# giesselmann/STRique

Measured on AMD Instinct MI355X. Metric: reads/s for STRique 'count' on 50 kb r9.4 signals, higher is better.
Workload: dtype f32

## Files before the change

strique_amd/csrc/screen_kernels.h:

```cpp
#pragma once
#include <hip/hip_runtime.h>
#include <stdint.h>
#include "align_kernels.h"

#define STRQ_SCREEN_R 14
#define STRQ_SCREEN_S 6
#define STRQ_SCREEN_SEG 4
#define STRQ_SCREEN_CHUNK_COLS 128
#define STRQ_SCREEN_MAX_WINDOWS 4
#define STRQ_SCREEN2_CPL 5
#define STRQ_SCREEN2_LPF 29
#define STRQ_SCREEN2_LANE_B 32

namespace strq {

struct ScreenParams {
    int32_t sc;
    int32_t hh, v;
    int32_t cadd;
    int32_t slack;
    int32_t merge_gap;
    int32_t max_cand;
    int32_t margin;
};

struct ScreenTask {
    const uint8_t* levels;
    const float* table;
    const int32_t* band_lo;
    int32_t* out;
    int32_t tsize;
    int32_t n, m, k, col_off;
    int32_t n_chunks;
    int32_t lane_last;
};

struct Screen2Task {
    const uint8_t* levels;
    const float* table[2];
    const int32_t* band_lo[2];
    int32_t* out[2];
    int32_t tsize[2], k[2];
    int32_t n, col_off, n_chunks;
};

struct ScreenWindows {
    int32_t n_win;
    int32_t lo[STRQ_SCREEN_MAX_WINDOWS], hi[STRQ_SCREEN_MAX_WINDOWS];
    float lower_bound;
    float upper_bound;
    int32_t n_cand;
};

int screen_plan(const AlignParams& p, int samples, int max_n, ScreenParams* sp);
static inline bool screen_flank_ok(int m) { return m >= 2 * STRQ_SCREEN_R && m <= 64 * STRQ_SCREEN_R; }
size_t screen_lds_bytes(int tsize);
int launch_screen(hipStream_t stream, const ScreenTask* tasks, int n_groups, int* queue, const ScreenParams& sp,
                  size_t lds_bytes, int tables_per_cu, int n_cu);
int screen2_plan(const AlignParams& p, int samples, int max_n, int merge, ScreenParams* sp);
static inline bool screen2_flank_ok(int m, int k) { return k >= 1 && k <= STRQ_SCREEN2_LPF * STRQ_SCREEN2_CPL && m == k * STRQ_SCREEN_S; }
size_t screen2_lds_bytes(int tsize_a, int tsize_b);
int launch_screen2(hipStream_t stream, const Screen2Task* tasks, int n_groups, int* queue, const ScreenParams& sp,
                   size_t lds_bytes, int groups_per_cu, int n_cu, int merge);
int launch_screen_windows(hipStream_t stream, const ScreenTask* tasks, int n_groups, const ScreenParams& sp,
                          const int32_t* bound_scaled, ScreenWindows* out, const int32_t* list = nullptr, const int32_t* theta_list = nullptr);

}
```

strique_amd/csrc/screen_kernels.hip:

```cpp
#include "strq_opt.h"
#include <hip/hip_runtime.h>
#include <stdint.h>
#include <stdlib.h>
#include <cmath>
#include "screen_kernels.h"

namespace strq {

namespace {

constexpr int R = STRQ_SCREEN_R, S = STRQ_SCREEN_S, SEG = STRQ_SCREEN_SEG;
constexpr int G = 2, C = 3;
static_assert(R == 14 && S == 6, "class expansion below is written for 14 rows per lane, 6 samples per class");

__device__ __forceinline__ int dpp_shr1(int v, int fill)
{
    return __builtin_amdgcn_update_dpp(fill, v, 0x138, 0xF, 0xF, false);
}
__device__ __forceinline__ int med3i(int a, int lo, int hi)
{
    int r;
    asm("v_med3_i32 %0, %1, %2, %3" : "=v"(r) : "v"(a), "v"(lo), "v"(hi));
    return r;
}
#define STRQ_SCREEN_BIAS 0x00800000
#ifndef STRQ_SCREEN_WPE
#define STRQ_SCREEN_WPE 6
#endif
__device__ __forceinline__ int max3i(int a, int b, int c)
{
    int r;
    asm("v_max3_f32 %0, %1, %2, %3" : "=v"(r) : "v"(a), "v"(b), "v"(c));
    return r;
}
__device__ __forceinline__ int sel_mask(int if0, int if1, uint64_t mask)
{
    int r;
    asm("v_cndmask_b32_e64 %0, %1, %2, %3" : "=v"(r) : "v"(if0), "v"(if1), "s"(mask));
    return r;
}

struct LaneConst { int lo2[C], hi2[C], off[C]; };

struct Screen {
    const char* lds;
    const LaneConst& lc;
    const uint64_t (&pm)[3];
    const int lane, n, hh;
    int T[R], SbotA, upS, potB, cmax;
    int qq;
    int scA[C], scB[C];

    __device__ __forceinline__ void fetch(int q2, int (&sc)[C])
    {
#pragma unroll
        for (int c = 0; c < C; ++c)
            sc[c] = *reinterpret_cast<const uint16_t*>(lds + med3i(q2, lc.lo2[c], lc.hi2[c]) + lc.off[c]);
    }
    __device__ __forceinline__ void advance(int qsrc, int snext, int& qn, int (&nA)[C], int (&nB)[C])
    {
        qn = __builtin_amdgcn_update_dpp(__builtin_amdgcn_readlane(qsrc, snext), qq, 0x138, 0xF, 0xF, false);
        fetch(qn & 0xffff, nA);
        fetch((int)((unsigned)qn >> 16), nB);
    }
    __device__ __forceinline__ void prime(int qcur)
    {
        qq = 0;
        int qn, nA[C], nB[C];
        advance(qcur, 0, qn, nA, nB);
        qq = qn;
#pragma unroll
        for (int c = 0; c < C; ++c) { scA[c] = nA[c]; scB[c] = nB[c]; }
    }
    __device__ __forceinline__ void expand(const int (&sc)[C], int (&rs)[R])
    {
#pragma unroll
        for (int r = 0; r < R; r += G) {
            const int base = r / S, x = (r % S) / G;
            int v;
            if (x == 0 || base + 1 >= C) v = sc[base < C ? base : C - 1];
            else v = sel_mask(sc[base], sc[base + 1], pm[x]);
#pragma unroll
            for (int g = 0; g < G && r + g < R; ++g) rs[r + g] = v;
        }
    }

    template <bool PRED>
    __device__ __forceinline__ void step(int t, int qsrc, int snext)
    {
        const int qn = __builtin_amdgcn_update_dpp(__builtin_amdgcn_readlane(qsrc, snext), qq, 0x138, 0xF, 0xF, false);
        const int potA = potB + hh, potBn = potA + hh;
        const int upA = dpp_shr1(SbotA, potA);
        const int upB = dpp_shr1(T[R - 1], potBn);
        int rsA[R], rsB[R];
        expand(scA, rsA);
        expand(scB, rsB);
        fetch(qn & 0xffff, scA);
        fetch((int)((unsigned)qn >> 16), scB);
        bool act = true, okB = true;
        if constexpr (PRED) { const int jB = 2 * (t - lane), jA = jB - 1; act = (jA >= 1) && (jA <= n); okB = jB <= n; }
        if (act) {
            int ta_prev = upA, ta_prev2 = upS, tb_prev2 = upB;
#pragma unroll
            for (int r = 0; r < R; ++r) {
                const int diagA = r == 0 ? upS : T[r - 1];
                const int ta = max3i(diagA + rsA[r], T[r], ta_prev);
                if (r > 0) {
                    const int tb = max3i(ta_prev2 + rsB[r - 1], ta_prev, tb_prev2);
                    T[r - 1] = tb; tb_prev2 = tb;
                }
                ta_prev2 = ta_prev; ta_prev = ta;
            }
            const int tb = max3i(ta_prev2 + rsB[R - 1], ta_prev, tb_prev2);
            T[R - 1] = tb;
            SbotA = ta_prev;
            upS = upB;
            const int cA = ta_prev - potA + STRQ_SCREEN_BIAS, cB = okB ? tb - potBn + STRQ_SCREEN_BIAS : cA;
            cmax = max3i(cmax, cA, cB);
        }
        potB = potBn;
        qq = qn;
    }
};

__device__ __forceinline__ int load_chunk(const ScreenTask& tk, int chunk, int lane)
{
    const int idx = (chunk * 64 + lane) * 2;
    int a = 0, b = 0;
    if (idx < tk.n) a = tk.levels[idx];
    if (idx + 1 < tk.n) b = tk.levels[idx + 1];
    return (a * 2) | ((b * 2) << 16);
}

}

size_t screen_lds_bytes(int tsize)
{
    return (size_t)((tsize + 1) & ~1) * 2 + 4;
}

__global__ void __attribute__((amdgpu_flat_work_group_size(64 * STRQ_SCREEN_SEG, 64 * STRQ_SCREEN_SEG), amdgpu_waves_per_eu(STRQ_SCREEN_WPE, STRQ_SCREEN_WPE)))
align_screen_kernel(const ScreenTask* __restrict__ tasks, int n_groups, int* __restrict__ queue, ScreenParams sp)
{
    extern __shared__ uint32_t lds_all[];
    __shared__ int next_group;
    const int lane = threadIdx.x & 63, wave = threadIdx.x >> 6;
    const char* ldsb = reinterpret_cast<const char*>(lds_all);
    for (;;) {
        __syncthreads();
        if (threadIdx.x == 0) next_group = atomicAdd(queue, 1);
        __syncthreads();
        const int gi = __builtin_amdgcn_readfirstlane(next_group);
        if (gi >= n_groups) break;
        const ScreenTask& t0 = tasks[(size_t)gi * SEG];
        const int ts = t0.tsize, zero_idx = (ts + 1) & ~1;
        {
            uint16_t* dst = reinterpret_cast<uint16_t*>(lds_all);
            const float scf = (float)sp.sc;
            for (int i = threadIdx.x; i < ts; i += 64 * SEG) dst[i] = (uint16_t)((int)ceilf(t0.table[i] * scf) + sp.cadd);
            if (threadIdx.x == 0) { dst[zero_idx] = 0; dst[zero_idx + 1] = 0; }
        }
        __syncthreads();
        const ScreenTask& tk = tasks[(size_t)gi * SEG + wave];
        if (tk.n <= 0) continue;

        LaneConst lc; uint64_t pm[3];
        {
            const int row0 = lane * R, kbase = row0 / S, phase = row0 % S;
#pragma unroll
            for (int c = 0; c < C; ++c) {
                const int k = kbase + c;
                if (k < tk.k) {
                    const uint32_t d = (uint32_t)tk.band_lo[k];
                    const int lo = (int)(d & 255u), w1 = (int)((d >> 8) & 255u), off = (int)(d >> 16);
                    lc.lo2[c] = lo * 2; lc.hi2[c] = (lo + w1) * 2;
                    lc.off[c] = (off - lo) * 2;
                } else {
                    lc.lo2[c] = 0; lc.hi2[c] = 0; lc.off[c] = zero_idx * 2;
                }
            }
            pm[0] = 0;
#pragma unroll
            for (int x = 1; x < 3; ++x) {
                const uint64_t b = __ballot(phase >= S - x * G);
                const uint32_t lo = __builtin_amdgcn_readfirstlane((int)(uint32_t)b), hi = __builtin_amdgcn_readfirstlane((int)(uint32_t)(b >> 32));
                pm[x] = ((uint64_t)hi << 32) | lo;
            }
        }
        const int lM = (tk.m - 1) / R;
        Screen f{ldsb, lc, pm, lane, tk.n, sp.hh};
        {
#pragma unroll
            for (int r = 0; r < R; ++r) f.T[r] = STRQ_SCREEN_BIAS;
            f.SbotA = STRQ_SCREEN_BIAS; f.upS = STRQ_SCREEN_BIAS;
            f.potB = STRQ_SCREEN_BIAS - 2 * lane * sp.hh;
            f.cmax = STRQ_SCREEN_BIAS;
        }
        const int nsteps = (tk.n + 1) / 2 + 63;
        int qcur = load_chunk(tk, 0, lane);
        f.prime(qcur);
        for (int t0s = 0; t0s < nsteps; t0s += 64) {
            const int qnext = load_chunk(tk, t0s / 64 + 1, lane);
            const bool full = (t0s >= 63) && (2 * (t0s + 64) <= tk.n);
            const int send = nsteps - t0s < 64 ? nsteps - t0s : 64;
            if (full) {
                for (int s = 0; s < 63; ++s) f.template step<false>(t0s + s + 1, qcur, s + 1);
                f.template step<false>(t0s + 64, qnext, 0);
            } else {
                for (int s = 0; s < send; ++s) {
                    const int qsrc = s == 63 ? qnext : qcur, snext = (s + 1) & 63;
                    f.template step<true>(t0s + s + 1, qsrc, snext);
                }
            }
            const int cm = __builtin_amdgcn_readlane(f.cmax, lM) - STRQ_SCREEN_BIAS;
            if (lane == 0) tk.out[t0s / 64] = cm;
            f.cmax = STRQ_SCREEN_BIAS;
            qcur = qnext;
        }
    }
}

namespace {

constexpr int CPL = STRQ_SCREEN2_CPL, LPF = STRQ_SCREEN2_LPF, LB = STRQ_SCREEN2_LANE_B;

struct Lane2Const { int lo2[CPL], hi2[CPL], off[CPL]; };

template <int RPC>
struct Screen2 {
    static constexpr int R2 = RPC * CPL;
    const char* lds;
    const Lane2Const& lc;
    const uint64_t top_mask;
    const int lane, n, hh;
    int T[R2], SbotA, upS, potB, cmax;
    int qq;
    int scA[CPL], scB[CPL];

    __device__ __forceinline__ int score(int q2, int c) const
    {
        return *reinterpret_cast<const uint16_t*>(lds + med3i(q2, lc.lo2[c], lc.hi2[c]) + lc.off[c]);
    }
    __device__ __forceinline__ void prime(int qcur)
    {
        qq = __builtin_amdgcn_update_dpp(__builtin_amdgcn_readlane(qcur, 0), 0, 0x138, 0xF, 0xF, false);
#pragma unroll
        for (int c = 0; c < CPL; ++c) { scA[c] = score(qq & 0xffff, c); scB[c] = score((int)((unsigned)qq >> 16), c); }
    }

    template <bool PRED>
    __device__ __forceinline__ void step(int t, int qsrc, int snext)
    {
        const int qn = __builtin_amdgcn_update_dpp(__builtin_amdgcn_readlane(qsrc, snext), qq, 0x138, 0xF, 0xF, false);
        const int qa = qn & 0xffff, qb = (int)((unsigned)qn >> 16);
        const int potA = potB + hh, potBn = potA + hh;
        const int upA = sel_mask(dpp_shr1(SbotA, potA), potA, top_mask);
        const int upB = sel_mask(dpp_shr1(T[R2 - 1], potBn), potBn, top_mask);
        bool act = true, okB = true;
        if constexpr (PRED) { const int jB = 2 * (t - lane), jA = jB - 1; act = (jA >= 1) && (jA <= n); okB = jB <= n; }
        int ta_prev = upA, ta_prev2 = upS;
        int tb_prev2 = upB;
#pragma unroll
        for (int c = 0; c < CPL; ++c) {
            if (act) {
#pragma unroll
                for (int r = RPC * c; r < RPC * c + RPC; ++r) {
                    const int diagA = r == 0 ? upS : T[r - 1];
                    const int ta = max3i(diagA + scA[c], T[r], ta_prev);
                    if (r > 0) {
                        const int tb = max3i(ta_prev2 + scB[(r - 1) / RPC], ta_prev, tb_prev2);
                        T[r - 1] = tb; tb_prev2 = tb;
                    }
                    ta_prev2 = ta_prev; ta_prev = ta;
                }
                if (c == CPL - 1) {
                    const int tb = max3i(ta_prev2 + scB[c], ta_prev, tb_prev2);
                    T[R2 - 1] = tb;
                    SbotA = ta_prev;
                    upS = upB;
                    const int cA = ta_prev - potA + STRQ_SCREEN_BIAS, cB = okB ? tb - potBn + STRQ_SCREEN_BIAS : cA;
                    cmax = max3i(cmax, cA, cB);
                }
            }
            scA[c] = score(qa, c);
            if (c > 0) scB[c - 1] = score(qb, c - 1);
            if (c == CPL - 1) scB[c] = score(qb, c);
        }
        potB = potBn;
        qq = qn;
    }
};

__device__ __forceinline__ int load_chunk2(const Screen2Task& tk, int chunk, int lane)
{
    const int idx = (chunk * 64 + lane) * 2;
    int a = 0, b = 0;
    if (idx < tk.n) a = tk.levels[idx];
    if (idx + 1 < tk.n) b = tk.levels[idx + 1];
    return (a * 2) | ((b * 2) << 16);
}

template <int RPC>
__device__ __forceinline__ void screen2_body(const Screen2Task* __restrict__ tasks, int n_groups, int* __restrict__ queue, const ScreenParams& sp)
{
    constexpr int R2 = RPC * CPL, MERGE = S / RPC;
    extern __shared__ uint32_t lds_all[];
    __shared__ int next_group;
    const int lane = threadIdx.x & 63, wave = threadIdx.x >> 6;
    const char* ldsb = reinterpret_cast<const char*>(lds_all);
    for (;;) {
        __syncthreads();
        if (threadIdx.x == 0) next_group = atomicAdd(queue, 1);
        __syncthreads();
        const int gi = __builtin_amdgcn_readfirstlane(next_group);
        if (gi >= n_groups) break;
        const Screen2Task& t0 = tasks[(size_t)gi * SEG];
        int base[2], zero_idx[2];
        base[0] = 0; zero_idx[0] = (t0.tsize[0] + 1) & ~1;
        base[1] = zero_idx[0] + 2; zero_idx[1] = base[1] + ((t0.tsize[1] + 1) & ~1);
        {
            uint16_t* dst = reinterpret_cast<uint16_t*>(lds_all);
            const float scf = (float)sp.sc;
#pragma unroll
            for (int f = 0; f < 2; ++f) {
                for (int i = threadIdx.x; i < t0.tsize[f]; i += 64 * SEG) dst[base[f] + i] = (uint16_t)(MERGE * ((int)ceilf(t0.table[f][i] * scf) + sp.cadd));
                if (threadIdx.x == 0) { dst[zero_idx[f]] = 0; dst[zero_idx[f] + 1] = 0; }
            }
        }
        __syncthreads();
        const Screen2Task& tk = tasks[(size_t)gi * SEG + wave];
        if (tk.n <= 0) continue;

        Lane2Const lc;
        const int f = lane >= LB ? 1 : 0, lf = lane - f * LB;
        {
#pragma unroll
            for (int c = 0; c < CPL; ++c) {
                const int k = lf * CPL + c;
                if (lf < LPF && k < tk.k[f]) {
                    const uint32_t d = (uint32_t)tk.band_lo[f][k];
                    const int lo = (int)(d & 255u), w1 = (int)((d >> 8) & 255u), off = (int)(d >> 16);
                    lc.lo2[c] = lo * 2; lc.hi2[c] = (lo + w1) * 2;
                    lc.off[c] = (base[f] + off - lo) * 2;
                } else {
                    lc.lo2[c] = 0; lc.hi2[c] = 0; lc.off[c] = zero_idx[f] * 2;
                }
            }
        }
        const uint64_t top_mask = 1ull | (1ull << LB);
        const int lMa = (tk.k[0] - 1) / CPL, lMb = LB + (tk.k[1] - 1) / CPL;
        Screen2<RPC> s2{ldsb, lc, top_mask, lane, tk.n, sp.hh};
        {
#pragma unroll
            for (int r = 0; r < R2; ++r) s2.T[r] = STRQ_SCREEN_BIAS;
            s2.SbotA = STRQ_SCREEN_BIAS; s2.upS = STRQ_SCREEN_BIAS;
            s2.potB = STRQ_SCREEN_BIAS - 2 * lane * sp.hh;
            s2.cmax = STRQ_SCREEN_BIAS;
        }
        const int nsteps = (tk.n + 1) / 2 + 63;
        int qcur = load_chunk2(tk, 0, lane);
        s2.prime(qcur);
        for (int t0s = 0; t0s < nsteps; t0s += 64) {
            const int qnext = load_chunk2(tk, t0s / 64 + 1, lane);
            const bool full = (t0s >= 63) && (2 * (t0s + 64) <= tk.n);
            const int send = nsteps - t0s < 64 ? nsteps - t0s : 64;
            if (full) {
                for (int s = 0; s < 63; ++s) s2.template step<false>(t0s + s + 1, qcur, s + 1);
                s2.template step<false>(t0s + 64, qnext, 0);
            } else {
                for (int s = 0; s < send; ++s) {
                    const int qsrc = s == 63 ? qnext : qcur, snext = (s + 1) & 63;
                    s2.template step<true>(t0s + s + 1, qsrc, snext);
                }
            }
            const int cma = __builtin_amdgcn_readlane(s2.cmax, lMa) - STRQ_SCREEN_BIAS;
            const int cmb = __builtin_amdgcn_readlane(s2.cmax, lMb) - STRQ_SCREEN_BIAS;
            if (lane == 0) { tk.out[0][t0s / 64] = cma; tk.out[1][t0s / 64] = cmb; }
            s2.cmax = STRQ_SCREEN_BIAS;
            qcur = qnext;
        }
    }
}

}

size_t screen2_lds_bytes(int tsize_a, int tsize_b)
{
    return (size_t)(((tsize_a + 1) & ~1) + 2 + ((tsize_b + 1) & ~1) + 2) * 2;
}

#define STRQ_SCREEN2_ATTR(WPE_) __attribute__((amdgpu_flat_work_group_size(64 * STRQ_SCREEN_SEG, 64 * STRQ_SCREEN_SEG), amdgpu_waves_per_eu(WPE_, WPE_)))
__global__ void STRQ_SCREEN2_ATTR(6) align_screen3_kernel(const Screen2Task* __restrict__ tasks, int n_groups, int* __restrict__ queue, ScreenParams sp) { screen2_body<2>(tasks, n_groups, queue, sp); }
__global__ void STRQ_SCREEN2_ATTR(4) align_screen1_kernel(const Screen2Task* __restrict__ tasks, int n_groups, int* __restrict__ queue, ScreenParams sp) { screen2_body<6>(tasks, n_groups, queue, sp); }

__global__ void __launch_bounds__(256)
screen_windows_kernel(const ScreenTask* __restrict__ tasks, int n_groups, ScreenParams sp,
                      const int32_t* __restrict__ bound_scaled, ScreenWindows* __restrict__ out,
                      const int32_t* __restrict__ list, const int32_t* __restrict__ theta_list)
{
    const int lane = threadIdx.x & 63;
    const int idx = blockIdx.x * (blockDim.x >> 6) + (threadIdx.x >> 6);
    if (idx >= n_groups) return;
    const int g = list ? list[idx] : idx;
    const ScreenTask* tg = tasks + (size_t)g * SEG;
    const int m = tg[0].m, lM = tg[0].lane_last;
    const int shift = -m * sp.v;
    int vmax = 0;
    for (int w = 0; w < SEG; ++w) {
        if (tg[w].n <= 0) continue;
        for (int c = lane; c < tg[w].n_chunks; c += 64) { const int v = tg[w].out[c]; vmax = v > vmax ? v : vmax; }
    }
#pragma unroll
    for (int d = 32; d >= 1; d >>= 1) { const int o = __shfl_xor(vmax, d, 64); vmax = o > vmax ? o : vmax; }
    ScreenWindows r;
    r.n_win = 0; r.n_cand = 0;
    for (int k = 0; k < STRQ_SCREEN_MAX_WINDOWS; ++k) { r.lo[k] = 0; r.hi[k] = 0; }
    const int drop = (sp.margin > 0 ? sp.margin : m) + 2 * sp.slack;
    int theta = theta_list ? theta_list[idx] : vmax - drop;
    if (!theta_list && sp.max_cand > 0) {
        auto count_at = [&](int t) {
            int n = 0;
            for (int w = 0; w < SEG; ++w) {
                if (tg[w].n <= 0) continue;
                for (int c = lane; c < tg[w].n_chunks; c += 64) n += tg[w].out[c] >= t;
            }
#pragma unroll
            for (int d = 32; d >= 1; d >>= 1) n += __shfl_xor(n, d, 64);
            return n;
        };
        if (count_at(theta) > sp.max_cand) {
            int lo = theta, hi = vmax;
            while (hi - lo > 1) {
                const int mid = lo + (hi - lo) / 2;
                if (count_at(mid) > sp.max_cand) lo = mid; else hi = mid;
            }
            theta = hi;
        }
    }
    r.upper_bound = (float)(vmax + shift + sp.slack) / (float)sp.sc;
    auto scan = [&](int th, bool store) -> int {
        int nw = 0, last_hi = -(1 << 30), ncand = 0;
        for (int w = 0; w < SEG; ++w) {
            if (tg[w].n <= 0) continue;
            for (int c0 = 0; c0 < tg[w].n_chunks; c0 += 64) {
                const int c1 = c0 + lane;
                const bool cand = c1 < tg[w].n_chunks && tg[w].out[c1] >= th;
                uint64_t mask = __ballot(cand);
                while (mask) {
                    const int bit = __builtin_ctzll(mask); mask &= mask - 1;
                    const int c = c0 + bit;
                    ++ncand;
                    int lo = 128 * c - 2 * lM + 1, hi = 128 * c - 2 * lM + 128;
                    if (lo < 1) lo = 1;
                    if (hi > tg[w].n) hi = tg[w].n;
                    if (hi < lo) continue;
                    lo += tg[w].col_off; hi += tg[w].col_off;
                    if (nw > 0 && lo <= last_hi + sp.merge_gap) {
                        if (hi > last_hi) last_hi = hi;
                        if (store) {
                            const int k = nw <= STRQ_SCREEN_MAX_WINDOWS ? nw - 1 : STRQ_SCREEN_MAX_WINDOWS - 1;
                            if (hi > r.hi[k]) r.hi[k] = hi;
                            if (lo < r.lo[k]) r.lo[k] = lo;
                        }
                    } else {
                        ++nw; last_hi = hi;
                        if (store) {
                            if (nw <= STRQ_SCREEN_MAX_WINDOWS) { r.lo[nw - 1] = lo; r.hi[nw - 1] = hi; }
                            else if (hi > r.hi[STRQ_SCREEN_MAX_WINDOWS - 1]) r.hi[STRQ_SCREEN_MAX_WINDOWS - 1] = hi;
                        }
                    }
                }
            }
        }
        if (store) r.n_cand = ncand;
        return nw;
    };
    if (!theta_list && sp.max_cand > 0 && scan(theta, false) > STRQ_SCREEN_MAX_WINDOWS) {
        int lo = theta, hi = vmax;
        while (hi - lo > 1) {
            const int mid = lo + (hi - lo) / 2;
            if (scan(mid, false) > STRQ_SCREEN_MAX_WINDOWS) lo = mid; else hi = mid;
        }
        theta = hi;
    }
    {
        const double lb = (double)(theta + shift + sp.slack) / (double)sp.sc;
        float lbf = (float)lb;
        if ((double)lbf < lb) {
            int32_t bits = __float_as_int(lbf);
            bits = lbf > 0.0f ? bits + 1 : (lbf < 0.0f ? bits - 1 : 1);
            lbf = __int_as_float(bits);
        }
        r.lower_bound = lbf;
    }
    const bool ok = theta + shift > 0 && theta + shift > bound_scaled[g];
    if (ok) {
        int nw = scan(theta, true);
        if (nw > STRQ_SCREEN_MAX_WINDOWS) nw = STRQ_SCREEN_MAX_WINDOWS;
        for (int a = 1; a < nw; ++a)
            for (int b = a; b > 0 && r.lo[b] < r.lo[b - 1]; --b) {
                const int tl = r.lo[b], th = r.hi[b]; r.lo[b] = r.lo[b - 1]; r.hi[b] = r.hi[b - 1]; r.lo[b - 1] = tl; r.hi[b - 1] = th;
            }
        int kept = nw > 0 ? 1 : 0;
        for (int a = 1; a < nw; ++a) {
            if (r.lo[a] <= r.hi[kept - 1] + 1) { if (r.hi[a] > r.hi[kept - 1]) r.hi[kept - 1] = r.hi[a]; }
            else { r.lo[kept] = r.lo[a]; r.hi[kept] = r.hi[a]; ++kept; }
        }
        for (int a = kept; a < STRQ_SCREEN_MAX_WINDOWS; ++a) { r.lo[a] = 0; r.hi[a] = 0; }
        r.n_win = kept;
    }
    if (lane == 0) out[idx] = r;
}

int screen_plan(const AlignParams& p, int samples, int max_n, ScreenParams* sp)
{
    if (strq::opt("STRQ_NO_SCREEN")) return 0;
    if (samples != S) return 0;
    if (!(p.open_h == p.ext_h && p.open_v == p.ext_v)) return 0;
    if (!(p.dist_min >= 0.0f) || !(p.ext_h < 0.0f) || !(p.ext_v < 0.0f) || !(p.dist_offset > 0.0f) || !(p.dist_min <= p.dist_offset)) return 0;
    for (int sc = 1024; sc >= 16; sc >>= 1) {
        const double hh = -(double)p.ext_h * sc, v = -(double)p.ext_v * sc, smax = std::ceil((double)p.dist_offset * sc);
        if (hh != (double)(long)hh || v != (double)(long)v) continue;
        if (hh < 1 || smax + v + hh > 65000.0) continue;
        const double top = 64.0 * R * (smax + v) + ((double)max_n + 256.0) * hh + smax + v + hh + (double)STRQ_SCREEN_BIAS;
        if (top > 2.0e9) continue;
        sp->sc = sc; sp->hh = (int)hh; sp->v = (int)v; sp->cadd = (int)(hh + v);
        {
            const double rows = 64.0 * R, maxval = rows * (double)p.dist_offset;
            double p2 = 1.0; while (p2 < maxval) p2 *= 2.0;
            const double adds = rows * (1.0 + (double)p.dist_offset / -(double)p.ext_h);
            const double e = adds * p2 / 16777216.0;
            if (!(e < 1.0e4)) continue;
            sp->slack = ((int)std::ceil(e) + 1) * sc;
        }
        sp->merge_gap = 3072; sp->margin = 0; sp->max_cand = 0;
        return 1;
    }
    return 0;
}

int screen2_plan(const AlignParams& p, int samples, int max_n, int merge, ScreenParams* sp)
{
    if (merge != 1 && merge != 3) return 0;
    if (!screen_plan(p, samples, max_n, sp)) return 0;
    while (sp->sc >= 16) {
        const double smax = std::ceil((double)p.dist_offset * sp->sc);
        if ((double)merge * (smax + sp->cadd) <= 65000.0) return 1;
        if ((sp->hh & 1) || (sp->v & 1)) return 0;
        sp->slack = (sp->slack / sp->sc) * (sp->sc / 2);
        sp->sc /= 2; sp->hh /= 2; sp->v /= 2; sp->cadd = sp->hh + sp->v;
    }
    return 0;
}

int launch_screen2(hipStream_t stream, const Screen2Task* tasks, int n_groups, int* queue, const ScreenParams& sp,
                   size_t lds_bytes, int groups_per_cu, int n_cu, int merge)
{
    if (n_groups <= 0) return 0;
    if (merge != 3 && merge != 1) return 2;
    auto kern = merge == 3 ? align_screen3_kernel : align_screen1_kernel;
    if (merge == 1 && groups_per_cu > 4) groups_per_cu = 4;
    if (groups_per_cu > 6) groups_per_cu = 6;
    (void)hipFuncSetAttribute((const void*)kern, hipFuncAttributeMaxDynamicSharedMemorySize, (int)lds_bytes);
    hipLaunchKernelGGL(kern, dim3(groups_per_cu * n_cu), dim3(64 * SEG), lds_bytes, stream, tasks, n_groups, queue, sp);
    return hipGetLastError() == hipSuccess ? 0 : 1;
}

int launch_screen(hipStream_t stream, const ScreenTask* tasks, int n_groups, int* queue, const ScreenParams& sp,
                  size_t lds_bytes, int tables_per_cu, int n_cu)
{
    if (n_groups <= 0) return 0;
    (void)hipFuncSetAttribute((const void*)align_screen_kernel, hipFuncAttributeMaxDynamicSharedMemorySize, (int)lds_bytes);
    hipLaunchKernelGGL(align_screen_kernel, dim3(tables_per_cu * n_cu), dim3(64 * SEG), lds_bytes, stream, tasks, n_groups, queue, sp);
    return hipGetLastError() == hipSuccess ? 0 : 1;
}

int launch_screen_windows(hipStream_t stream, const ScreenTask* tasks, int n_groups, const ScreenParams& sp,
                          const int32_t* bound_scaled, ScreenWindows* out, const int32_t* list, const int32_t* theta_list)
{
    if (n_groups <= 0) return 0;
    hipLaunchKernelGGL(screen_windows_kernel, dim3((n_groups + 3) / 4), dim3(256), 0, stream, tasks, n_groups, sp, bound_scaled, out, list, theta_list);
    return hipGetLastError() == hipSuccess ? 0 : 1;
}

}
```

strique_amd/csrc/strq_align_api.hip:

```cpp
#include <hip/hip_runtime.h>
#include <algorithm>
#include <cmath>
#include <climits>
#include <cstring>
#include <cstdlib>
#include <time.h>
#include <unistd.h>
#include <map>
#include <mutex>
#include <string>
#include <tuple>
#include <numeric>
#include <vector>
#include "../../include/strique_hip.h"
#include "strq_ctx.h"
#include "align_kernels.h"
#include "lut_kernels.h"
#include "align_generic.h"

using namespace strq;

#define STRQ_DBG(...) do { if (strq::opt("STRQ_DEBUG")) { fprintf(stderr, "[strq] " __VA_ARGS__); fprintf(stderr, "\n"); fflush(stderr); } } while (0)

namespace strq {

static thread_local const strq_ctx* t_cur_ctx = nullptr;
static std::mutex g_opt_mu;
static std::map<std::string, std::string> g_opts;
CtxScope::CtxScope(const strq_ctx* c) : prev(t_cur_ctx) { t_cur_ctx = c; }
CtxScope::~CtxScope() { t_cur_ctx = prev; }
const char* opt(const char* key)
{
    static thread_local std::string ring[8];
    static thread_local unsigned ring_pos = 0;
    auto keep = [&](const std::string& v) -> const char* {
        if (v.empty()) return nullptr;
        std::string& slot = ring[ring_pos++ & 7u];
        slot = v;
        return slot.c_str();
    };
    if (t_cur_ctx) {
        std::lock_guard<std::mutex> lk(t_cur_ctx->options_mu);
        auto it = t_cur_ctx->options.find(key);
        if (it != t_cur_ctx->options.end()) return keep(it->second);
    }
    {
        std::lock_guard<std::mutex> lk(g_opt_mu);
        auto it = g_opts.find(key);
        if (it != g_opts.end()) return keep(it->second);
    }
    return getenv(key);
}

float host_cell_score(const AlignParams& p, float h, float v)
{
    const float d = h > v ? h - v : v - h;
    const float s = p.dist_offset - (float)std::pow((double)d, 1.2);
    return s > p.dist_min ? s : p.dist_min;
}

void host_col0(const AlignParams& p, int m, float* out)
{
    const float NINF = -3.4028234663852886e38f / 2;
    out[0] = 0.0f;
    float vprev = NINF, sprev = 0.0f;
    for (int i = 1; i <= m; ++i) {
        const float ext = vprev + p.ext_v, opn = sprev + p.open_v;
        const float v = ext >= opn ? ext : opn;
        out[i] = v; vprev = v; sprev = v;
    }
}

struct BatchIn {
    int64_t n_align, n_reads;
    const uint8_t* levels; const int64_t* read_off; const float* level_val;
    const int32_t* align_read; const float* flank; const int64_t* flank_off; int32_t samples;
};
struct BatchOut { float* score; int64_t* j_end; int64_t* j0; int32_t* rec; };


static const int hard_cap = 1 << 16;
static const int trace_wpb = 8;

struct Piece { int col_off, n; size_t ck; };

static int cut(int n, int segs, int ov, Piece* out)
{
    int use = segs;
    while (use > 1 && (ov <= 0 || (long)n < (long)(use + 1) * ov)) --use;
    const long len = use > 1 ? ((long)n + (long)(use - 1) * ov + use - 1) / use : n;
    long o = 0;
    for (int k = 0; k < segs; ++k) {
        if (k >= use) { out[k].col_off = 0; out[k].n = 0; continue; }
        const long start = k == 0 ? 0 : o - ov;
        long end = k == use - 1 ? n : start + len; if (end > n) end = n;
        out[k].col_off = (int)start; out[k].n = (int)(end - start);
        o = end;
    }
    return use;
}

static int packed_dwords(int entries) { return (((2 * entries + 3) & ~3) + entries + 3) / 4; }

struct Launch { int R, NS, tables, first, count, first_task, first_up, lds_floats, packed, segs; bool known_last_row; };

struct CorePlan {
    CorePlan(strq_ctx* c_, const AlignCoreIn& in_, AlignCoreOut& out_) : c(c_), in(in_), out(out_), nb(in_.nb), S(in_.samples), st(c_->stream) {}
    strq_ctx* c;
    const AlignCoreIn& in;
    AlignCoreOut& out;
    const int nb, S;
    const hipStream_t st;

    bool collapsed = false, allow_pack = false, ov_fixed = false, scr_forced = false, mode_fine = false, mode_coarse = false;
    int seg_want = 0, max_tables = 8, max_waves = 16, ov_cap = 8192;
    std::map<std::pair<int, int>, int> ov_of_m;

    std::vector<size_t> cls_off, col0_off, bnd_off;
    std::vector<int> J0, NJ;
    std::vector<int> job_align, job_k0, job_k;
    std::vector<size_t> tab_off, desc_off;
    int nj = 0, max_k = 0;
    std::vector<float> h_cls;
    std::vector<LutJob> jobs;
    std::vector<LutInfo> info;
    std::vector<int> tab_total;

    std::vector<ScreenWindows> wins;
    bool screen2_ran = false;
    std::vector<int> g2_of;
    ScreenTask* d_st2 = nullptr;
    int32_t* d_bound2 = nullptr;
    ScreenParams sp2{};
    double coarse_cols = 0, coarse_all = 0;

    std::vector<char> packed;
    std::vector<int> overlap, segs_of;
    std::vector<Launch> launches;
    int n_up = 0, max_ns = 1, r2_cap = 0, qi = STRQ_QUEUE_FIRST;
    size_t n_tasks = 0, safe0 = 0, r2_0 = 0;
    std::vector<Piece> pieces, safe;
    std::vector<float> min_score;
    std::vector<char> two_round;
    bool any_two_round = false;
    std::vector<size_t> ck_up;
    std::vector<AlignTask> tasks;
    AlignTask *d_tasks = nullptr, *d_heads = nullptr;
    AlignResult *d_seg = nullptr, *d_res = nullptr, *d_seg_safe = nullptr;
    int32_t* d_pick = nullptr;
    float* d_min_score = nullptr;
    int *d_redo = nullptr, *d_redo_count = nullptr;
};

static int overlap_for(CorePlan& p, int m, int ov_worst, int redo_weight = 1)
{
    strq_ctx* c = p.c;
    if (p.ov_fixed || c->score_fracs.size() < 64 || c->mean_n <= 0) return std::min(ov_worst, p.ov_cap);
    auto it = p.ov_of_m.find(std::make_pair(m, redo_weight));
    if (it != p.ov_of_m.end()) return it->second;
    const std::vector<float>& f = c->score_fracs;
    double best_cost = 0; int best_ov = std::min(ov_worst, p.ov_cap);
    for (int ov = 1024; ; ov += 512) {
        if (ov > ov_worst) ov = ov_worst;
        const float need = align_segment_min_score(c->ap, m, ov) / ((float)m * c->ap.dist_offset) + 0.01f;
        const double redo = (double)(std::lower_bound(f.begin(), f.end(), need) - f.begin()) / (double)f.size();
        const double cost = 3.0 * ov / c->mean_n + redo_weight * redo * (1.0 + 3.0 * ov_worst / c->mean_n);
        if (best_cost == 0 || cost < best_cost) { best_cost = cost; best_ov = ov; }
        if (ov >= ov_worst) break;
    }
    p.ov_of_m[std::make_pair(m, redo_weight)] = best_ov;
    STRQ_DBG("overlap for %d-row flanks: %d columns (worst case %d; previous sub-batch: median score fraction %.3f, mean read %.0f samples)", m, best_ov, ov_worst, f[f.size() / 2], c->mean_n);
    return best_ov;
}

static int tables_for(const CorePlan& p, int dwords, int segs)
{
    int t = std::min(p.max_tables, (160 * 1024 - 64) / (std::max(dwords, 1) * 4));
    if (segs > 1) t = std::min(t, p.max_waves / segs);
    return t;
}

static void pause_after_fail(int& pause, int& fail)
{
    pause = std::min(256, 8 << std::min(fail, 5));
    ++fail;
}

static int upload_inputs(CorePlan& p)
{
    strq_ctx* c = p.c; const AlignCoreIn& in = p.in; AlignCoreOut& out = p.out;
    const int nb = p.nb, S = p.S;
    hipStream_t st = p.st;
    size_t cls_tot = 0, col0_tot = 0, rec_tot = 0, tab_tot = 0, bnd_floats = 0, desc_tot = 0;
    p.cls_off.assign(nb, 0); p.col0_off.assign(nb, 0); p.bnd_off.assign(nb, 0);
    std::map<const float*, size_t> cls_of_flank; std::map<int, size_t> col0_of_m;
    std::vector<int> cls_first, col0_first;
    out.rec_off.assign(nb, 0);
    p.J0.assign(nb, 0); p.NJ.assign(nb, 0);
    for (int i = 0; i < nb; ++i) {
        auto fc = cls_of_flank.find(in.flank[i]);
        if (fc == cls_of_flank.end()) { fc = cls_of_flank.emplace(in.flank[i], cls_tot).first; cls_tot += in.k[i]; cls_first.push_back(i); }
        p.cls_off[i] = fc->second;
        auto f0 = col0_of_m.find(in.m[i]);
        if (f0 == col0_of_m.end()) { f0 = col0_of_m.emplace(in.m[i], col0_tot).first; col0_tot += in.m[i] + 1; col0_first.push_back(i); }
        p.col0_off[i] = f0->second;
        p.J0[i] = (int)p.job_align.size();
        p.NJ[i] = in.k[i] > STRQ_LUT_MAX_K ? in.NS[i] : 1;
        for (int sidx = 0; sidx < p.NJ[i]; ++sidx) {
            int k0 = 0, kn = in.k[i];
            if (p.NJ[i] > 1) {
                const int row0 = sidx * 64 * in.R[i], rows = std::min(64 * in.R[i], in.m[i] - row0);
                k0 = row0 / S; kn = (row0 + rows - 1) / S - k0 + 1;
            }
            p.job_align.push_back(i); p.job_k0.push_back(k0); p.job_k.push_back(kn);
            p.desc_off.push_back(desc_tot); desc_tot += kn;
            p.tab_off.push_back(tab_tot); tab_tot += STRQ_TABLE_SLOT_FLOATS(kn);
            p.max_k = std::max(p.max_k, kn);
        }
        out.rec_off[i] = rec_tot; rec_tot += in.m[i];
        p.bnd_off[i] = bnd_floats; if (in.NS[i] > 1) bnd_floats += (size_t)(in.NS[i] - 1) * 2 * ((size_t)in.n[i] + 2);
    }
    const int nj = p.nj = (int)p.job_align.size();
    out.rec_total = rec_tot;
    p.h_cls.assign(cls_tot, 0.0f);
    std::vector<float> h_col0(col0_tot);
    for (int i : cls_first) {
        const float* f = in.flank[i];
        for (int kk = 0; kk < in.k[i]; ++kk) p.h_cls[p.cls_off[i] + kk] = f[(size_t)kk * S];
    }
    for (int i : col0_first) host_col0(c->ap, in.m[i], &h_col0[p.col0_off[i]]);
    STRQ_HIP(c, c->flank_cls.reserve(cls_tot * 4));
    STRQ_HIP(c, c->col0.reserve(col0_tot * 4));
    STRQ_HIP(c, c->band_lo.reserve(desc_tot * 4));
    STRQ_HIP(c, c->tables.reserve(tab_tot * 4));
    STRQ_HIP(c, c->tables3.reserve(tab_tot * 3 + (size_t)nj * 8 + 64));
    STRQ_HIP(c, c->bnd.reserve(bnd_floats * 4 + 256));
    STRQ_HIP(c, c->rec.reserve(rec_tot * 4 + 256));
    STRQ_HIP(c, c->lutinfo.reserve((size_t)nj * (sizeof(LutJob) + sizeof(LutInfo))));
    STRQ_HIP(c, c->hard.reserve((size_t)hard_cap * (sizeof(HardEntry) + 4) + 64));
    STRQ_HIP(c, c->queue.reserve(STRQ_QUEUE_BYTES));
    STRQ_HIP(c, hipMemcpyAsync(c->flank_cls.p, p.h_cls.data(), cls_tot * 4, hipMemcpyHostToDevice, st));
    STRQ_HIP(c, hipMemcpyAsync(c->col0.p, h_col0.data(), col0_tot * 4, hipMemcpyHostToDevice, st));
    STRQ_HIP(c, hipMemsetAsync(c->queue.p, 0, STRQ_QUEUE_BYTES, st));
    return STRQ_OK;
}

static int build_tables(CorePlan& p)
{
    strq_ctx* c = p.c; const AlignCoreIn& in = p.in;
    const int nb = p.nb, nj = p.nj;
    hipStream_t st = p.st;
    std::vector<LutJob>& jobs = p.jobs;
    std::vector<LutInfo>& info = p.info;
    jobs.resize(nj);
    LutJob* d_jobs = c->lutinfo.as<LutJob>();
    LutInfo* d_info = reinterpret_cast<LutInfo*>(d_jobs + nj);
    for (int j = 0; j < nj; ++j) {
        const int i = p.job_align[j];
        jobs[j].level_val = in.d_level_val + (size_t)in.read[i] * 256;
        jobs[j].cls_val = c->flank_cls.as<float>() + p.cls_off[i] + p.job_k0[j];
        jobs[j].table = c->tables.as<float>() + p.tab_off[j];
        jobs[j].table3 = c->tables3.as<uint8_t>() + p.tab_off[j] * 3 + (size_t)j * 8 - (p.tab_off[j] * 3 + (size_t)j * 8) % 4;
        jobs[j].band_lo = c->band_lo.as<int32_t>() + p.desc_off[j];
        jobs[j].k = p.job_k[j]; jobs[j].pad_ = 0;
    }
    STRQ_HIP(c, hipMemcpyAsync(d_jobs, jobs.data(), (size_t)nj * sizeof(LutJob), hipMemcpyHostToDevice, st));
    HardEntry* d_hard = c->hard.as<HardEntry>();
    float* d_hard_vals = reinterpret_cast<float*>(d_hard + hard_cap);
    int* d_hard_count = c->queue.as<int>();
    STRQ_HIP(c, hipEventRecord(c->ev[0], st));
    if (launch_lut_build(st, d_jobs, d_info, nj, p.max_k, d_hard, d_hard_count, hard_cap, c->ap)) { c->err = "lut launch failed"; return STRQ_ERR_DEVICE; }
    STRQ_HIP(c, hipEventRecord(c->ev[1], st));
    if (in.after_tables) { const int arc = in.after_tables(); if (arc) return arc; }
    info.resize(nj);
    int hard_count = 0;
    STRQ_HIP(c, hipMemcpyAsync(info.data(), d_info, (size_t)nj * sizeof(LutInfo), hipMemcpyDeviceToHost, st));
    STRQ_HIP(c, hipMemcpyAsync(&hard_count, d_hard_count, 4, hipMemcpyDeviceToHost, st));
    STRQ_HIP(c, hipStreamSynchronize(st));
    STRQ_DBG("lut done nb=%d hard=%d floats0=%d", nb, hard_count, info[0].total);
    if (strq::opt("STRQ_DEBUG")) { int hist[9] = {0}; for (int i = 0; i < nj; ++i) hist[std::min(8, info[i].need / 8)]++; STRQ_DBG("band need histogram (x8 levels): %d %d %d %d %d %d %d %d %d", hist[0], hist[1], hist[2], hist[3], hist[4], hist[5], hist[6], hist[7], hist[8]); }
    if (strq::opt("STRQ_DEBUG")) { long tot = 0; int mx = 0; for (int i = 0; i < nj; ++i) { tot += info[i].total; mx = std::max(mx, info[i].total); } STRQ_DBG("table floats: mean %.0f max %d (k=%d)", (double)tot / nj, mx, in.k[0]); }
    if (hard_count > hard_cap) { c->err = "too many borderline table entries"; return STRQ_ERR_DEVICE; }
    bool any_rebuild = false;
    for (int j = 0; j < nj; ++j) any_rebuild |= info[j].n_hard < 0;
    auto level_vals_of = [&](int read, float* dst) -> int {
        STRQ_HIP(c, hipMemcpy(dst, in.d_level_val + (size_t)read * 256, 256 * 4, hipMemcpyDeviceToHost));
        return STRQ_OK;
    };
    if (hard_count > 0) {
        std::vector<HardEntry> he(hard_count); std::vector<float> hv(hard_count);
        STRQ_HIP(c, hipMemcpy(he.data(), d_hard, (size_t)hard_count * sizeof(HardEntry), hipMemcpyDeviceToHost));
        float lv[256]; int last_read = -1;
        for (int i = 0; i < hard_count; ++i) {
            const int rd = in.read[p.job_align[he[i].job]];
            if (rd != last_read) { const int rc = level_vals_of(rd, lv); if (rc) return rc; last_read = rd; }
            hv[i] = host_cell_score(c->ap, lv[he[i].level], p.h_cls[p.cls_off[p.job_align[he[i].job]] + p.job_k0[he[i].job] + he[i].k]);
        }
        STRQ_HIP(c, hipMemcpyAsync(d_hard_vals, hv.data(), (size_t)hard_count * 4, hipMemcpyHostToDevice, st));
        if (launch_lut_patch(st, d_jobs, d_hard, d_hard_vals, hard_count)) { c->err = "patch launch failed"; return STRQ_ERR_DEVICE; }
        STRQ_HIP(c, hipStreamSynchronize(st));
    }
    if (any_rebuild) for (int j = 0; j < nj; ++j) if (info[j].n_hard < 0) {
        const int kk = p.job_k[j], i = p.job_align[j];
        std::vector<float> tab((size_t)kk * 256); std::vector<int32_t> blo(kk);
        float lv[256];
        { const int rc = level_vals_of(in.read[i], lv); if (rc) return rc; }
        for (int x = 0; x < kk; ++x) {
            float* row = &tab[(size_t)x * 256];
            for (int q = 0; q < 256; ++q) row[q] = host_cell_score(c->ap, lv[q], p.h_cls[p.cls_off[i] + p.job_k0[j] + x]);
            blo[x] = (int32_t)((255u << 8) | ((uint32_t)(x * 256) << 16));
        }
        STRQ_HIP(c, hipMemcpy(jobs[j].table, tab.data(), tab.size() * 4, hipMemcpyHostToDevice));
        STRQ_HIP(c, hipMemcpy(jobs[j].band_lo, blo.data(), (size_t)kk * 4, hipMemcpyHostToDevice));
        info[j].total = kk * 256;
    }
    p.tab_total.assign(nb, 0);
    for (int j = 0; j < nj; ++j) p.tab_total[p.job_align[j]] = std::max(p.tab_total[p.job_align[j]], info[j].total);
    p.out.n_hard = hard_count;
    return STRQ_OK;
}

static void read_switches(CorePlan& p)
{
    const strq_ctx* c = p.c;
    p.collapsed = p.S == 6 && c->ap.open_h == c->ap.ext_h && c->ap.open_v == c->ap.ext_v;
    if (const char* e = strq::opt("STRQ_SEG")) { const int v = atoi(e); if (v >= 1 && v <= 4) p.seg_want = v; }
    if (const char* e = strq::opt("STRQ_TABLES")) { const int v = atoi(e); if (v >= 1 && v <= 8) p.max_tables = v; }
    if (const char* e = strq::opt("STRQ_MAX_WAVES")) { const int v = atoi(e); if (v >= 4 && v <= 16) p.max_waves = v; }
    p.allow_pack = p.collapsed && !strq::opt("STRQ_NO_PACK");
    if (const char* e = strq::opt("STRQ_OVERLAP")) { const int v = atoi(e); p.ov_cap = v > 0 ? v : (1 << 30); p.ov_fixed = true; }
    p.scr_forced = strq::opt("STRQ_SCREEN_ALWAYS") != nullptr;
    const char* mode_opt = strq::opt("STRQ_SCREEN_MODE");
    p.mode_fine = mode_opt && std::strcmp(mode_opt, "fine") == 0;
    p.mode_coarse = mode_opt && std::strcmp(mode_opt, "coarse") == 0;
}


struct ScreenJob {
    int flanks = 1;
    std::vector<int> al;
    std::vector<ScreenTask> views;
    std::vector<Screen2Task> t2;
    std::vector<int32_t> bound;
    std::vector<size_t> out_off;
    size_t out_words = 0, lds_bytes = 0;
    double steps = 0;
};

struct ScreenRules {
    int merge;
    int groups_per_cu;
    const char* lds_err;
    bool below_bound_free;
    bool count_untaken;
    bool judge;
    double max_cols;
    int* pause; int* fail;
};

static void screen_tasks(CorePlan& p, const ScreenParams& sp, ScreenJob& j)
{
    constexpr int SSEG = STRQ_SCREEN_SEG;
    const AlignCoreIn& in = p.in;
    const int F = j.flanks, ng = (int)j.al.size() / F;
    if (F == 2) j.t2.resize((size_t)ng * SSEG);
    j.views.resize(j.al.size() * SSEG);
    j.bound.resize(j.al.size());
    j.out_off.assign(j.al.size() * SSEG, 0);
    for (int g = 0; g < ng; ++g) {
        const int* a = &j.al[(size_t)g * F];
        const int n = in.n[a[0]];
        const int m_big = F == 2 ? std::max(in.m[a[0]], in.m[a[1]]) : in.m[a[0]];
        const int ov_worst = align_segment_overlap(p.c->ap, m_big), ov_s = overlap_for(p, m_big, ov_worst, 16);
        Piece pc[SSEG];
        const int used = cut(n, SSEG, ov_s, pc);
        j.lds_bytes = std::max(j.lds_bytes, F == 2 ? screen2_lds_bytes(p.info[p.J0[a[0]]].total, p.info[p.J0[a[1]]].total) : screen_lds_bytes(p.info[p.J0[a[0]]].total));
        for (int f = 0; f < F; ++f)
            j.bound[(size_t)g * F + f] = used <= 1 ? INT32_MIN / 2 : (ov_s >= ov_worst ? 0 : (int32_t)std::ceil((double)align_segment_min_score(p.c->ap, in.m[a[f]], ov_s) * sp.sc));
        for (int w = 0; w < SSEG; ++w) {
            Screen2Task t; std::memset(&t, 0, sizeof(t));
            t.levels = in.d_levels + in.read_off[in.read[a[0]]] + pc[w].col_off;
            t.n = pc[w].n; t.col_off = pc[w].col_off;
            t.n_chunks = pc[w].n > 0 ? (align_num_steps(pc[w].n) + 63) / 64 : 0;
            for (int f = 0; f < F; ++f) {
                const LutJob& job = p.jobs[p.J0[a[f]]];
                t.table[f] = job.table; t.band_lo[f] = job.band_lo; t.tsize[f] = p.info[p.J0[a[f]]].total; t.k[f] = in.k[a[f]];
                ScreenTask v; std::memset(&v, 0, sizeof(v));
                v.n = pc[w].n; v.m = in.m[a[f]]; v.k = in.k[a[f]]; v.col_off = pc[w].col_off; v.n_chunks = t.n_chunks;
                if (F == 2) v.lane_last = f * STRQ_SCREEN2_LANE_B + (in.k[a[f]] - 1) / STRQ_SCREEN2_CPL;
                else { v.levels = t.levels; v.table = t.table[0]; v.band_lo = t.band_lo[0]; v.tsize = t.tsize[0]; v.lane_last = (v.m - 1) / STRQ_SCREEN_R; }
                j.out_off[((size_t)g * F + f) * SSEG + w] = j.out_words; j.out_words += (size_t)t.n_chunks;
                j.views[((size_t)g * F + f) * SSEG + w] = v;
            }
            if (pc[w].n > 0) j.steps += align_num_steps(pc[w].n);
            if (F == 2) j.t2[(size_t)g * SSEG + w] = t;
        }
    }
}

static int run_screen(CorePlan& p, ScreenJob& j, const ScreenParams& sp, const ScreenRules& r)
{
    constexpr int SSEG = STRQ_SCREEN_SEG;
    strq_ctx* c = p.c; const AlignCoreIn& in = p.in;
    hipStream_t st = p.st;
    const int nv = (int)j.al.size();
    if (j.lds_bytes > 160 * 1024 - 64) { c->err = r.lds_err; return STRQ_ERR_UNSUPPORTED; }
    const int groups = std::max(1, std::min(r.groups_per_cu, (int)((160 * 1024 - 64) / j.lds_bytes)));
    auto aligned = [](size_t bytes) { return (bytes + 255) & ~(size_t)255; };
    const size_t t2_bytes = aligned(j.t2.size() * sizeof(Screen2Task)), task_bytes = aligned(j.views.size() * sizeof(ScreenTask));
    const size_t bound_bytes = aligned((size_t)nv * 4), win_bytes = aligned((size_t)nv * sizeof(ScreenWindows));
    STRQ_HIP(c, c->screen.reserve(t2_bytes + task_bytes + bound_bytes + win_bytes + j.out_words * 4 + 256));
    char* base = c->screen.as<char>();
    Screen2Task* d_t2 = reinterpret_cast<Screen2Task*>(base);
    ScreenTask* d_st = reinterpret_cast<ScreenTask*>(base + t2_bytes);
    int32_t* d_bound = reinterpret_cast<int32_t*>(base + t2_bytes + task_bytes);
    ScreenWindows* d_win = reinterpret_cast<ScreenWindows*>(base + t2_bytes + task_bytes + bound_bytes);
    int32_t* d_out = reinterpret_cast<int32_t*>(base + t2_bytes + task_bytes + bound_bytes + win_bytes);
    for (size_t x = 0; x < j.views.size(); ++x) j.views[x].out = d_out + j.out_off[x];
    if (j.flanks == 2)
        for (int v = 0; v < nv; ++v) for (int w = 0; w < SSEG; ++w) j.t2[(size_t)(v / 2) * SSEG + w].out[v % 2] = j.views[(size_t)v * SSEG + w].out;
    if (j.flanks == 2) STRQ_HIP(c, hipMemcpyAsync(d_t2, j.t2.data(), j.t2.size() * sizeof(Screen2Task), hipMemcpyHostToDevice, st));
    STRQ_HIP(c, hipMemcpyAsync(d_st, j.views.data(), j.views.size() * sizeof(ScreenTask), hipMemcpyHostToDevice, st));
    STRQ_HIP(c, hipMemcpyAsync(d_bound, j.bound.data(), (size_t)nv * 4, hipMemcpyHostToDevice, st));
    STRQ_HIP(c, hipEventRecord(c->ev[5], st));
    int* queue = c->queue.as<int>() + STRQ_QUEUE_FIRST - 1;
    if (j.flanks == 2) {
        if (launch_screen2(st, d_t2, nv / 2, queue, sp, j.lds_bytes, groups, c->n_cu, r.merge)) { c->err = "coarse screen launch failed"; return STRQ_ERR_DEVICE; }
    } else {
        if (launch_screen(st, d_st, nv, queue, sp, j.lds_bytes, groups, c->n_cu)) { c->err = "screen launch failed"; return STRQ_ERR_DEVICE; }
    }
    STRQ_HIP(c, hipEventRecord(c->ev[6], st));
    if (launch_screen_windows(st, d_st, nv, sp, d_bound, d_win)) { c->err = "screen windows launch failed"; return STRQ_ERR_DEVICE; }
    std::vector<ScreenWindows> hw((size_t)nv);
    STRQ_HIP(c, hipMemcpyAsync(hw.data(), d_win, hw.size() * sizeof(ScreenWindows), hipMemcpyDeviceToHost, st));
    STRQ_HIP(c, hipStreamSynchronize(st));
    c->screen_ran = true; c->screen_mode_last = r.merge > 1 ? 2 : 1; c->coarse_merge_last = r.merge;
    if (const char* path = strq::opt("STRQ_SCREEN_DUMP")) {
        std::vector<int32_t> ho(j.out_words);
        STRQ_HIP(c, hipMemcpy(ho.data(), d_out, j.out_words * 4, hipMemcpyDeviceToHost));
        if (FILE* fp = fopen(path, "wb")) {
            const int32_t hdr[8] = {nv, sp.sc, sp.hh, sp.v, j.flanks, SSEG, sp.slack, r.merge};
            fwrite(hdr, 4, 8, fp);
            for (int v = 0; v < nv; ++v) {
                const int32_t gh[4] = {j.al[v], j.al[v], j.bound[v], j.views[(size_t)v * SSEG].lane_last};
                fwrite(gh, 4, 4, fp);
                for (int w = 0; w < SSEG; ++w) {
                    const ScreenTask& t = j.views[(size_t)v * SSEG + w];
                    const int32_t th[4] = {t.col_off, t.n, t.m, t.n_chunks};
                    fwrite(th, 4, 4, fp);
                    fwrite(ho.data() + (t.out - d_out), 4, (size_t)t.n_chunks, fp);
                }
                fwrite(&hw[(size_t)v], sizeof(ScreenWindows), 1, fp);
            }
            fclose(fp);
        }
    }
    if (const char* e = strq::opt("STRQ_SCREEN_TEST_RAISE")) {
        const float up = (float)atof(e);
        for (auto& w : hw) w.lower_bound += up;
    }
    int windowed = 0, heavy = 0, below_bound = 0; double cols = 0, all = 0;
    for (int v = 0; v < nv; ++v) {
        const int al = j.al[v];
        const ScreenWindows& w = hw[(size_t)v];
        c->screen_stats[1] += 1; c->screen_stats[7] += w.n_cand;
        double mine = in.n[al];
        if (w.n_win > 0) {
            p.wins[al] = w; c->screen_stats[2] += 1; ++windowed; mine = 0;
            for (int k = 0; k < w.n_win; ++k) { c->screen_stats[4] += w.hi[k] - w.lo[k] + 1; mine += w.hi[k] - w.lo[k] + 1 + 4096; }
        } else {
            c->screen_stats[3] += 1;
            if (w.n_cand == 0) { ++below_bound; if (r.below_bound_free) mine = 0; }
        }
        all += in.n[al]; cols += mine; heavy += mine > 4 * 32768.0;
    }
    if (r.count_untaken) c->screen_stats[3] += p.nb - nv;
    c->screen_stats[5] += j.steps; c->screen_stats[6] = sp.sc;
    if (j.flanks == 2) {
        p.screen2_ran = true;
        p.d_st2 = d_st; p.d_bound2 = d_bound; p.sp2 = sp;
        for (int v = 0; v < nv; ++v) p.g2_of[j.al[v]] = v;
        p.coarse_cols = cols; p.coarse_all = all;
    }
    if (r.judge && nv >= 64) {
        if (below_bound * 10 > nv && !p.ov_fixed) c->score_fracs.clear();
        else if (windowed < 0.9 * (nv - (p.ov_fixed ? 0 : below_bound)) || cols > r.max_cols * all || (long)heavy * 100 > 2L * nv) pause_after_fail(*r.pause, *r.fail);
        else *r.fail = 0;
    }
    STRQ_DBG("screen (%d flanks per wave, merge %d): %d alignments, scale %d, margin %.0f, %d groups per CU, LDS %zu bytes: %d with windows (%d below the cold-start bound), %.2f %% of the columns, %d heavy -> pause %d",
             j.flanks, r.merge, nv, sp.sc, (double)sp.margin / sp.sc, groups, j.lds_bytes, windowed, below_bound, 100.0 * cols / std::max(1.0, all), heavy, *r.pause);
    return STRQ_OK;
}

static int screen_two_flank(CorePlan& p, int merge, int max_n)
{
    strq_ctx* c = p.c; const AlignCoreIn& in = p.in;
    const int nb = p.nb;
    ScreenParams sp;
    if (!screen2_plan(c->ap, p.S, max_n, merge, &sp)) return STRQ_OK;
    const bool fine_rules = merge == 1;
    int min_n = fine_rules ? 65536 : 28672, groups = 6;
    if (const char* e = strq::opt("STRQ_SCREEN_MIN_N")) min_n = atoi(e);
    if (const char* e = strq::opt("STRQ_SCREEN2_GROUPS")) { const int v = atoi(e); if (v >= 1 && v <= 8) groups = v; }
    std::map<int, std::vector<int>> by_read;
    for (int i = 0; i < nb; ++i)
        if (in.NS[i] == 1 && p.NJ[i] == 1 && in.n[i] >= min_n && screen2_flank_ok(in.m[i], in.k[i])) by_read[in.read[i]].push_back(i);
    std::vector<std::pair<int, int>> pairs;
    for (auto& kv : by_read) {
        const std::vector<int>& v = kv.second;
        if (v.size() == 2) { pairs.emplace_back(v[0], v[1]); continue; }
        for (size_t x = 0; x + 1 < v.size(); ++x)
            if (!(v[x] & 1) && v[x + 1] == v[x] + 1) { pairs.emplace_back(v[x], v[x + 1]); ++x; }
    }
    std::stable_sort(pairs.begin(), pairs.end(), [&](const std::pair<int, int>& x, const std::pair<int, int>& y) { return in.n[x.first] > in.n[y.first]; });
    const int ngr = (int)pairs.size();
    if (ngr == 0 || 2 * ngr < (nb * 9) / 10) return STRQ_OK;
    sp.margin = (int32_t)std::lround((double)c->coarse_margin * (merge == 3 ? 1.3 : 1.0) * sp.sc);
    if (const char* e = strq::opt("STRQ_SCREEN2_MARGIN")) sp.margin = (int32_t)std::lround(atof(e) * sp.sc);
    sp.max_cand = 8;
    if (const char* e = strq::opt("STRQ_SCREEN2_MAX_CAND")) sp.max_cand = atoi(e);
    if (fine_rules) { sp.margin = 0; sp.max_cand = 0; }
    ScreenJob j;
    j.flanks = 2;
    for (const auto& pr : pairs) { j.al.push_back(pr.first); j.al.push_back(pr.second); }
    screen_tasks(p, sp, j);
    ScreenRules r;
    r.merge = merge; r.groups_per_cu = groups;
    r.lds_err = "score tables do not fit LDS (coarse screen)";
    r.below_bound_free = !p.ov_fixed; r.count_untaken = true;
    if (fine_rules) { r.judge = !p.scr_forced; r.max_cols = 0.15; r.pause = &c->screen_pause; r.fail = &c->screen_fail; }
    else { r.judge = !p.mode_coarse && !p.scr_forced; r.max_cols = 0.30; r.pause = &c->coarse_pause; r.fail = &c->coarse_fail; }
    return run_screen(p, j, sp, r);
}

static int screen_one_flank(CorePlan& p, const ScreenParams& sp)
{
    strq_ctx* c = p.c; const AlignCoreIn& in = p.in;
    int min_n = 65536;
    if (const char* e = strq::opt("STRQ_SCREEN_MIN_N")) min_n = atoi(e);
    std::vector<int> sel;
    for (int i = 0; i < p.nb; ++i)
        if (in.NS[i] == 1 && p.NJ[i] == 1 && in.n[i] >= min_n && screen_flank_ok(in.m[i]) && in.k[i] * p.S == in.m[i]) sel.push_back(i);
    std::stable_sort(sel.begin(), sel.end(), [&](int x, int y) { return in.n[x] > in.n[y]; });
    if (sel.empty()) return STRQ_OK;
    ScreenJob j;
    j.al = sel;
    screen_tasks(p, sp, j);
    ScreenRules r;
    r.merge = 0; r.groups_per_cu = 6;
    r.lds_err = "score table does not fit LDS (screen)";
    r.below_bound_free = false; r.count_untaken = false;
    r.judge = true; r.max_cols = 0.10; r.pause = &c->screen_pause; r.fail = &c->screen_fail;
    return run_screen(p, j, sp, r);
}

static int run_screens(CorePlan& p)
{
    strq_ctx* c = p.c; const AlignCoreIn& in = p.in;
    const int nb = p.nb;
    p.wins.resize(nb);
    c->screen_ran = false;
    STRQ_HIP(c, hipEventRecord(c->ev[2], p.st));
    int max_n = 0;
    for (int i = 0; i < nb; ++i) max_n = std::max(max_n, in.n[i]);
    c->screen_mode_last = 0;
    const int coarse_merge = 3;
    p.g2_of.assign(nb, -1);
    for (int attempt = 0; attempt < 2 && !p.screen2_ran; ++attempt) {
        int merge = coarse_merge;
        if (attempt == 0) {
            if (!p.collapsed || p.mode_fine || strq::opt("STRQ_NO_SCREEN")) continue;
            if (c->coarse_pause > 0 && !p.mode_coarse && !p.scr_forced) { --c->coarse_pause; continue; }
        } else {
            if (!p.collapsed || strq::opt("STRQ_NO_SCREEN") || (c->screen_pause > 0 && !p.scr_forced)) continue;
            merge = 1;
        }
        const int rc = screen_two_flank(p, merge, max_n);
        if (rc) return rc;
    }
    if (p.screen2_ran) return STRQ_OK;
    if (p.collapsed && c->screen_pause > 0 && !p.scr_forced) {
        --c->screen_pause; c->screen_stats[3] += nb;
        return STRQ_OK;
    }
    ScreenParams sp;
    if (p.collapsed && screen_plan(c->ap, p.S, max_n, &sp)) return screen_one_flank(p, sp);
    return STRQ_OK;
}

static int plan_launches(CorePlan& p)
{
    strq_ctx* c = p.c; const AlignCoreIn& in = p.in; AlignCoreOut& out = p.out;
    const int nb = p.nb;
    std::vector<ScreenWindows>& wins = p.wins;
    static const double rate[5][2] = {{0, 0}, {1.017, 0.941}, {0.79, 0.862}, {0.85, 0.85}, {0.69, 0.80}};
    p.packed.assign(nb, 0); p.overlap.assign(nb, 0); p.segs_of.assign(nb, 1);
    std::vector<char> segmentable(nb, 0);
    const bool force_pack = strq::opt("STRQ_PACK") != nullptr;
    int class_count[5] = {0, 0, 0, 0, 0};
    for (int i = 0; i < nb; ++i) {
        segmentable[i] = p.collapsed && in.NS[i] == 1;
        p.overlap[i] = segmentable[i] ? align_segment_overlap(c->ap, in.m[i]) : 0;
        const bool can_pack = p.allow_pack && in.NS[i] == 1 && p.info[p.J0[i]].packed && p.info[p.J0[i]].n_hard == 0;
        int best_s = 1, best_p = can_pack ? 1 : 0;
        if (segmentable[i]) {
            const double l = overlap_for(p, in.m[i], p.overlap[i]);
            double best_cost = 0;
            for (int sgs : {1, 2, 3, 4}) {
                if (p.seg_want ? sgs != p.seg_want : sgs == 3) continue;
                if (sgs > 1 && !p.seg_want && (l <= 0 || in.n[i] < (sgs + 1) * l)) continue;
                for (int pk = 0; pk < 2; ++pk) {
                    if ((pk && !can_pack) || (force_pack && can_pack && !pk)) continue;
                    const double cost = (in.n[i] + (sgs - 1) * l) * rate[sgs][pk];
                    if (best_cost == 0 || cost < best_cost) { best_cost = cost; best_s = sgs; best_p = pk; }
                }
            }
        }
        if (wins[i].n_win > 0) {
            ScreenWindows& w = wins[i];
            while (w.n_win < STRQ_SCREEN_MAX_WINDOWS) {
                int widest = 0;
                for (int k2 = 1; k2 < w.n_win; ++k2) if (w.hi[k2] - w.lo[k2] > w.hi[widest] - w.lo[widest]) widest = k2;
                if (w.hi[widest] - w.lo[widest] < 16384) break;
                const int mid = w.lo[widest] + (w.hi[widest] - w.lo[widest]) / 2;
                for (int k2 = w.n_win; k2 > widest + 1; --k2) { w.lo[k2] = w.lo[k2 - 1]; w.hi[k2] = w.hi[k2 - 1]; }
                w.lo[widest + 1] = mid + 1; w.hi[widest + 1] = w.hi[widest]; w.hi[widest] = mid;
                ++w.n_win;
            }
            const int nw = w.n_win;
            best_s = p.seg_want >= nw ? p.seg_want : (nw <= 2 ? nw : 4); best_p = 0;
        }
        p.segs_of[i] = best_s; p.packed[i] = (char)best_p;
        ++class_count[best_s];
    }
    std::vector<int>& segs_of = p.segs_of;
    if (!p.seg_want && !c->screen_ran) {
        int few = 2 * c->n_cu;
        if (const char* e = strq::opt("STRQ_CLASS_MIN")) few = atoi(e);
        if (class_count[4] && class_count[4] < few) { for (int i = 0; i < nb; ++i) if (segs_of[i] == 4) { segs_of[i] = 2; if (wins[i].n_win > 2) wins[i].n_win = 0; } class_count[2] += class_count[4]; class_count[4] = 0; }
        if (class_count[2] && class_count[2] < few && class_count[1]) { for (int i = 0; i < nb; ++i) if (segs_of[i] == 2) { segs_of[i] = 1; if (wins[i].n_win > 1) wins[i].n_win = 0; } class_count[1] += class_count[2]; class_count[2] = 0; }
    }
    std::map<std::tuple<int, int, int, int, int>, std::vector<int>> groups;
    for (int i = 0; i < nb; ++i) {
        const int w = tables_for(p, p.packed[i] ? packed_dwords(p.tab_total[i]) : p.tab_total[i], segs_of[i]);
        if (w < 1) { c->err = "score table does not fit LDS"; return STRQ_ERR_UNSUPPORTED; }
        groups[std::make_tuple(in.R[i], in.NS[i], -segs_of[i], -w, p.packed[i] ? 0 : 1)].push_back(i);
    }
    const int min_rounds = 4;
    for (auto it = groups.begin(); it != groups.end();) {
        auto nx = std::next(it);
        const int w = -std::get<3>(it->first);
        const bool same_kind = nx != groups.end() && std::get<0>(nx->first) == std::get<0>(it->first) && std::get<1>(nx->first) == std::get<1>(it->first)
                               && std::get<2>(nx->first) == std::get<2>(it->first)
                               && !(std::get<4>(it->first) == 1 && std::get<4>(nx->first) == 0);
        if (same_kind && (long)it->second.size() < (long)min_rounds * w * c->n_cu) {
            nx->second.insert(nx->second.end(), it->second.begin(), it->second.end());
            it = groups.erase(it);
        } else ++it;
    }
    out.order.clear(); out.order.reserve(nb);
    for (auto& g : groups) {
        auto& v = g.second;
        auto work = [&](int x) {
            if (wins[x].n_win <= 0) return (long)in.n[x];
            long w = 0;
            for (int k = 0; k < wins[x].n_win; ++k) w += wins[x].hi[k] - wins[x].lo[k] + 1 + 4096;
            return w;
        };
        std::stable_sort(v.begin(), v.end(), [&](int x, int y) { return work(x) > work(y); });
        const int NS = std::get<1>(g.first);
        const int pk = std::get<4>(g.first) == 0;
        int lds_floats = 0;
        for (int i : v) lds_floats = std::max(lds_floats, pk ? packed_dwords(p.tab_total[i]) : p.tab_total[i]);
        const int segs = -std::get<2>(g.first);
        const int tables = std::min(-std::get<3>(g.first), tables_for(p, lds_floats, segs));
        if (tables < 1) { c->err = "score table does not fit LDS"; return STRQ_ERR_UNSUPPORTED; }
        bool known = std::get<0>(g.first) == 14;
        for (int i : v) known = known && in.m[i] == 870;
        p.launches.push_back({std::get<0>(g.first), NS, tables, (int)out.order.size(), (int)v.size(), (int)p.n_tasks, 0, lds_floats, pk, segs, known});
        out.order.insert(out.order.end(), v.begin(), v.end());
        p.n_tasks += (size_t)v.size() * segs;
        if (NS > 1) p.n_up += (int)v.size() * (NS - 1);
    }
    { size_t up = p.n_tasks; for (auto& L : p.launches) if (L.NS > 1) { L.first_up = (int)up; up += (size_t)L.count * (L.NS - 1); } }
    return STRQ_OK;
}

static int cut_pieces(CorePlan& p)
{
    strq_ctx* c = p.c; const AlignCoreIn& in = p.in; const AlignCoreOut& out = p.out;
    const int nb = p.nb;
    const size_t n_tasks = p.n_tasks;
    p.safe0 = n_tasks + p.n_up + (size_t)nb;
    p.pieces.resize(n_tasks); p.safe.resize(n_tasks);
    p.min_score.assign(nb, -INFINITY);
    p.two_round.assign(p.launches.size(), 0);
    p.ck_up.assign(nb, 0);
    size_t ck_floats = 0;
    for (size_t li = 0; li < p.launches.size(); ++li) {
        auto& L = p.launches[li];
        for (int x = 0; x < L.count; ++x) {
            const int pos = L.first + x, i = out.order[pos];
            const int n = in.n[i], R = in.R[i], ov = p.overlap[i];
            const size_t per_ckpt = (size_t)STRQ_CKPT_FIELDS(R) * 64;
            Piece* pf = &p.pieces[(size_t)L.first_task + (size_t)x * L.segs];
            Piece* ps = &p.safe[(size_t)L.first_task + (size_t)x * L.segs];
            cut(n, L.segs, ov, ps);
            const int ov_fast = overlap_for(p, in.m[i], ov);
            if (p.wins[i].n_win > 0) {
                const ScreenWindows& w = p.wins[i];
                const int ov_w = std::min(ov > 0 ? ov : (1 << 30), align_overlap_for_score(c->ap, in.m[i], w.lower_bound));
                for (int k = 0; k < L.segs; ++k) {
                    if (k < w.n_win) { const int start = std::max(0, w.lo[k] - 1 - ov_w); pf[k].col_off = start; pf[k].n = w.hi[k] - start; }
                    else { pf[k].col_off = 0; pf[k].n = 0; }
                }
                p.min_score[pos] = std::max(w.lower_bound, align_segment_min_score(c->ap, in.m[i], ov_w));
                p.two_round[li] = 1;
            } else if (L.segs > 1 && ov_fast < ov && cut(n, L.segs, ov_fast, pf) > 1) {
                p.min_score[pos] = align_segment_min_score(c->ap, in.m[i], ov_fast);
                p.two_round[li] = 1;
            } else {
                for (int k = 0; k < L.segs; ++k) pf[k] = ps[k];
            }
            for (int k = 0; k < L.segs; ++k) {
                pf[k].ck = ps[k].ck = ck_floats;
                ck_floats += (size_t)align_num_ckpts(std::max(pf[k].n, ps[k].n)) * per_ckpt;
            }
            if (L.NS > 1) { p.ck_up[i] = ck_floats; ck_floats += (size_t)(L.NS - 1) * align_num_ckpts(n) * per_ckpt; }
        }
    }
    for (char t : p.two_round) p.any_two_round |= t != 0;
    const size_t n_all_tasks = p.safe0 + (p.any_two_round ? n_tasks : 0);
    STRQ_HIP(c, c->ckpt.reserve(ck_floats * 4 + 256));
    p.r2_cap = p.screen2_ran ? std::max(1024, std::min(nb, 8192)) : 0;
    p.r2_0 = n_all_tasks;
    STRQ_HIP(c, c->tasks.reserve((n_all_tasks + (size_t)p.r2_cap * 4) * sizeof(AlignTask)));
    STRQ_HIP(c, c->results.reserve((2 * n_tasks + nb) * sizeof(AlignResult) + (size_t)nb * 12 + p.launches.size() * 4 + 256));
    p.tasks.resize(n_all_tasks);
    p.d_tasks = c->tasks.as<AlignTask>();
    p.d_heads = p.d_tasks + n_tasks + p.n_up;
    p.d_seg = c->results.as<AlignResult>();
    p.d_res = p.d_seg + n_tasks;
    p.d_seg_safe = p.d_res + nb;
    p.d_pick = reinterpret_cast<int32_t*>(p.d_seg_safe + n_tasks);
    p.d_min_score = reinterpret_cast<float*>(p.d_pick + nb);
    p.d_redo = reinterpret_cast<int*>(p.d_min_score + nb);
    p.d_redo_count = p.d_redo + nb;
    return STRQ_OK;
}

static int write_tasks(CorePlan& p)
{
    strq_ctx* c = p.c; const AlignCoreIn& in = p.in; AlignCoreOut& out = p.out;
    const int nb = p.nb, S = p.S;
    hipStream_t st = p.st;
    const size_t n_tasks = p.n_tasks, n_up = p.n_up, safe0 = p.safe0;
    std::vector<AlignTask>& tasks = p.tasks;
    for (auto& L : p.launches) {
        for (int x = 0; x < L.count; ++x) {
            const int pos = L.first + x, i = out.order[pos];
            const int R = in.R[i], M = in.m[i];
            AlignTask base; std::memset(&base, 0, sizeof(base));
            base.levels = in.d_levels + in.read_off[in.read[i]];
            base.rec = c->rec.as<int32_t>() + out.rec_off[i];
            base.n = in.n[i]; base.n_full = in.n[i]; base.m_total = M;
            auto strip = [&](int row0, int rows, size_t ck, int sidx) {
                AlignTask t = base;
                const int j = p.NJ[i] > 1 ? p.J0[i] + sidx : p.J0[i];
                const int k0 = row0 / S, k1 = (row0 + rows - 1) / S;
                t.row0 = row0; t.m = rows; t.k = k1 - k0 + 1; t.tsize = p.info[j].total;
                t.table = p.jobs[j].table; t.table3 = p.jobs[j].table3; t.band_lo = p.jobs[j].band_lo + (k0 - p.job_k0[j]);
                t.col0 = c->col0.as<float>() + p.col0_off[i] + row0;
                t.ckpt = c->ckpt.as<float>() + ck;
                return t;
            };
            tasks[n_tasks + n_up + pos] = strip(0, M, 0, 0);
            if (L.NS == 1) {
                for (int k = 0; k < L.segs; ++k) {
                    const size_t ti = (size_t)L.first_task + (size_t)x * L.segs + k;
                    AlignTask t = strip(0, M, p.pieces[ti].ck, 0);
                    t.levels += p.pieces[ti].col_off; t.n = p.pieces[ti].n; t.col_off = p.pieces[ti].col_off;
                    tasks[ti] = t;
                    if (p.any_two_round) {
                        AlignTask u = strip(0, M, p.safe[ti].ck, 0);
                        u.levels += p.safe[ti].col_off; u.n = p.safe[ti].n; u.col_off = p.safe[ti].col_off;
                        tasks[safe0 + ti] = u;
                    }
                }
            } else {
                const int rows_s = 64 * R;
                const size_t ck_strip = (size_t)align_num_ckpts(in.n[i]) * STRQ_CKPT_FIELDS(R) * 64;
                float* bnd = c->bnd.as<float>() + p.bnd_off[i];
                const size_t bnd_stride = 2 * ((size_t)in.n[i] + 2);
                for (int sidx = 0; sidx < L.NS; ++sidx) {
                    const bool last = sidx == L.NS - 1;
                    const int row0 = sidx * rows_s, rows = last ? M - row0 : rows_s;
                    const size_t slot = last ? (size_t)L.first_task + x : (size_t)L.first_up + (size_t)sidx * L.count + x;
                    AlignTask t = strip(row0, rows, last ? p.pieces[(size_t)L.first_task + x].ck : p.ck_up[i] + (size_t)sidx * ck_strip, sidx);
                    if (sidx > 0) { t.bnd_in = bnd + (size_t)(sidx - 1) * bnd_stride; t.up = p.d_tasks + L.first_up + (size_t)(sidx - 1) * L.count + x; }
                    if (!last) t.bnd_out = bnd + (size_t)sidx * bnd_stride;
                    tasks[slot] = t;
                    if (last && p.any_two_round) tasks[safe0 + slot] = t;
                }
            }
        }
    }
    STRQ_HIP(c, hipMemcpyAsync(p.d_tasks, tasks.data(), tasks.size() * sizeof(AlignTask), hipMemcpyHostToDevice, st));
    STRQ_HIP(c, hipMemsetAsync(p.d_seg, 0, (2 * n_tasks + nb) * sizeof(AlignResult), st));
    if (p.any_two_round) {
        STRQ_HIP(c, hipMemcpyAsync(p.d_min_score, p.min_score.data(), (size_t)nb * 4, hipMemcpyHostToDevice, st));
        STRQ_HIP(c, hipMemsetAsync(p.d_redo_count, 0, p.launches.size() * 4, st));
    }
    size_t scratch_words = 0;
    for (auto& L : p.launches) scratch_words = std::max(scratch_words, align_trace_scratch_words_per_wave(L.R));
    STRQ_HIP(c, c->scratch.reserve(scratch_words * 8 * (size_t)c->n_cu * trace_wpb));
    out.n_launches = 0; out.wave_steps = 0; out.columns = 0;
    for (size_t t = 0; t < n_tasks + n_up; ++t) if (tasks[t].n > 0) { out.wave_steps += align_num_steps(tasks[t].n); out.columns += tasks[t].n; }
    if (!p.launches.empty()) {
        const Launch& L = p.launches.back(); out.segs = L.segs; out.tables = L.tables; out.packed = L.packed; out.rows_per_lane = L.R;
        const int i = out.order[L.first];
        out.overlap_worst = p.overlap[i]; out.overlap_first = L.segs > 1 ? overlap_for(p, in.m[i], p.overlap[i]) : 0;
        const bool seg_kernel = L.NS == 1 && p.collapsed;
        const int32_t g[8] = {L.segs, L.tables, seg_kernel ? align_segments_wpe(L.segs, L.tables) : 0, L.R, L.packed, out.overlap_first, out.overlap_worst, (int32_t)p.launches.size()};
        std::memcpy(c->geometry, g, sizeof(g));
    }
    return STRQ_OK;
}

static int run_forward(CorePlan& p)
{
    strq_ctx* c = p.c; AlignCoreOut& out = p.out;
    const int S = p.S;
    hipStream_t st = p.st;
    const std::vector<Launch>& launches = p.launches;
    for (auto& L : launches) p.max_ns = std::max(p.max_ns, L.NS);
    if ((size_t)STRQ_QUEUE_FIRST + launches.size() * ((size_t)p.max_ns + 2) + 16 > (size_t)STRQ_QUEUE_SLOTS) {
        c->err = "too many distinct (flank shape, table size) groups in one batch"; return STRQ_ERR_UNSUPPORTED;
    }
    bool side = false;
    std::vector<hipStream_t> lstream(launches.size(), st);
    if (c->screen_ran && launches.size() > 1 && p.max_ns == 1 && p.collapsed) {
        side = true;
        if (!c->ev_fork) STRQ_HIP(c, hipEventCreateWithFlags(&c->ev_fork, hipEventDisableTiming));
        STRQ_HIP(c, hipEventRecord(c->ev_fork, st));
        size_t biggest = 0;
        for (size_t li = 1; li < launches.size(); ++li) if (launches[li].count > launches[biggest].count) biggest = li;
        if (!c->side_stream) { STRQ_HIP(c, hipStreamCreateWithFlags(&c->side_stream, hipStreamNonBlocking)); STRQ_HIP(c, hipEventCreateWithFlags(&c->side_join, hipEventDisableTiming)); }
        STRQ_HIP(c, hipStreamWaitEvent(c->side_stream, c->ev_fork, 0));
        lstream[biggest] = c->side_stream;
    }
    for (int level = 0; level < p.max_ns; ++level) {
        for (size_t lidx = 0; lidx < launches.size(); ++lidx) {
            const Launch& L = launches[lidx];
            hipStream_t lst = lstream[lidx];
            if (level >= L.NS) continue;
            STRQ_DBG("forward launch R=%d strips=%d slice dwords=%d packed=%d level=%d count=%d tables/CU=%d segments=%d", L.R, L.NS, L.lds_floats, L.packed, level, L.count, L.tables, L.segs);
            int rc;
            if (L.NS == 1 && p.collapsed) {
                rc = launch_align_segments(lst, L.R, S, p.d_tasks + L.first_task, p.d_seg + L.first_task, L.count, L.segs, c->queue.as<int>() + p.qi,
                                           c->ap, L.lds_floats, L.tables, c->n_cu, L.packed, nullptr, nullptr, L.known_last_row);
            } else {
                const bool last = level == L.NS - 1;
                const AlignTask* dt = last ? p.d_tasks + L.first_task : p.d_tasks + L.first_up + (size_t)level * L.count;
                const int mode = (level > 0 ? 1 : 0) | (last ? 0 : 2);
                rc = launch_align(st, L.R, S, dt, p.d_seg + L.first_task, L.count, c->queue.as<int>() + p.qi, c->ap, L.lds_floats, L.tables, c->n_cu,
                                  c->scratch.as<uint64_t>(), 0, mode, L.packed);
            }
            if (rc) { c->err = "align launch failed"; return STRQ_ERR_DEVICE; }
            ++p.qi; ++out.n_launches;
        }
    }
    if (side) {
        STRQ_HIP(c, hipEventRecord(c->side_join, c->side_stream));
        STRQ_HIP(c, hipStreamWaitEvent(st, c->side_join, 0));
    }
    for (size_t li = 0; li < launches.size(); ++li) {
        const Launch& L = launches[li];
        int* redo = p.d_redo + L.first; int* cnt = p.d_redo_count + li;
        if (launch_align_combine(st, p.d_tasks + L.first_task, p.d_seg + L.first_task, L.count, L.segs, p.d_res + L.first, p.d_pick + L.first, L.first_task,
                                 nullptr, nullptr, p.two_round[li] ? p.d_min_score + L.first : nullptr, redo, cnt,
                                 c->redo_total.p ? c->redo_total.as<unsigned int>() : nullptr)) { c->err = "combine launch failed"; return STRQ_ERR_DEVICE; }
    }
    return STRQ_OK;
}

struct Look2 { int pos, i, g2; float b1; };

static void keep_whole_read(const CorePlan& p, std::vector<std::vector<int>>& redo_keep, int pos)
{
    for (size_t li = 0; li < p.launches.size(); ++li) {
        const Launch& L = p.launches[li];
        if (pos >= L.first && pos < L.first + L.count) redo_keep[li].push_back(pos - L.first);
    }
}

static int look2_run(CorePlan& p, const std::vector<Look2>& l2, std::vector<std::vector<int>>& redo_keep)
{
    strq_ctx* c = p.c; const AlignCoreIn& in = p.in; AlignCoreOut& out = p.out;
    const int nb = p.nb, S = p.S;
    hipStream_t st = p.st;
    const ScreenParams& sp2 = p.sp2;
    const int n2 = (int)l2.size();
    const size_t o_list = 0, o_theta = o_list + (size_t)n2 * 4, o_win = (o_theta + (size_t)n2 * 4 + 15) & ~(size_t)15,
                 o_pos = o_win + (size_t)n2 * sizeof(ScreenWindows), o_seg = (o_pos + (size_t)n2 * 4 + 15) & ~(size_t)15,
                 o_res = o_seg + (size_t)n2 * 4 * sizeof(AlignResult), o_pick = o_res + (size_t)n2 * sizeof(AlignResult), o_end = o_pick + (size_t)n2 * 4;
    STRQ_HIP(c, c->misc.reserve(o_end + 256));
    char* mb = c->misc.as<char>();
    std::vector<int32_t> h_list((size_t)n2), h_theta((size_t)n2), h_pos((size_t)n2);
    for (int k2 = 0; k2 < n2; ++k2) {
        const Look2& e = l2[(size_t)k2];
        h_list[(size_t)k2] = e.g2; h_pos[(size_t)k2] = e.pos;
        const double b1s = std::floor((double)e.b1 * sp2.sc);
        h_theta[(size_t)k2] = (int32_t)std::max(-2.0e9, std::min(2.0e9, b1s + (double)in.m[e.i] * sp2.v - (double)sp2.slack));
    }
    STRQ_HIP(c, hipMemcpyAsync(mb + o_list, h_list.data(), (size_t)n2 * 4, hipMemcpyHostToDevice, st));
    STRQ_HIP(c, hipMemcpyAsync(mb + o_theta, h_theta.data(), (size_t)n2 * 4, hipMemcpyHostToDevice, st));
    STRQ_HIP(c, hipMemcpyAsync(mb + o_pos, h_pos.data(), (size_t)n2 * 4, hipMemcpyHostToDevice, st));
    if (launch_screen_windows(st, p.d_st2, n2, sp2, p.d_bound2, reinterpret_cast<ScreenWindows*>(mb + o_win),
                              reinterpret_cast<const int32_t*>(mb + o_list), reinterpret_cast<const int32_t*>(mb + o_theta))) { c->err = "screen windows launch failed"; return STRQ_ERR_DEVICE; }
    std::vector<ScreenWindows> w2((size_t)n2);
    STRQ_HIP(c, hipMemcpyAsync(w2.data(), mb + o_win, (size_t)n2 * sizeof(ScreenWindows), hipMemcpyDeviceToHost, st));
    STRQ_HIP(c, hipStreamSynchronize(st));
    std::map<int, std::vector<int>> by_R;
    for (int k2 = 0; k2 < n2; ++k2) {
        if (w2[(size_t)k2].n_win > 0) by_R[in.R[l2[(size_t)k2].i]].push_back(k2);
        else keep_whole_read(p, redo_keep, l2[(size_t)k2].pos);
    }
    const int piece_cols = 8192;
    std::vector<AlignTask> t2; t2.reserve((size_t)n2 * 4);
    std::vector<int32_t> pos_sorted, grp_first;
    size_t ck2 = 0; int slot = 0, n_grp = 0; double cols2 = 0;
    struct G2 { int R, first_grp, n_grp, lds, tables; bool known; };
    std::vector<G2> groups2;
    const size_t r2_task_cap = (size_t)p.r2_cap * 4;
    for (auto& kv : by_R) {
        G2 g{kv.first, n_grp, 0, 0, 0, kv.first == 14};
        for (int k2 : kv.second) {
            const Look2& e = l2[(size_t)k2];
            const ScreenWindows& w = w2[(size_t)k2];
            const int ov = p.overlap[e.i];
            const int ov_w = std::min(ov > 0 ? ov : (1 << 30), align_overlap_for_score(c->ap, in.m[e.i], w.lower_bound));
            int need = 0;
            for (int q = 0; q < w.n_win; ++q) need += (w.hi[q] - w.lo[q] + piece_cols) / piece_cols;
            need = (need + 3) & ~3;
            if (t2.size() + (size_t)need > r2_task_cap) { keep_whole_read(p, redo_keep, e.pos); continue; }
            const AlignTask& head = p.tasks[p.n_tasks + p.n_up + (size_t)e.pos];
            const size_t per_ckpt = (size_t)STRQ_CKPT_FIELDS(in.R[e.i]) * 64;
            int made = 0;
            for (int q = 0; q < w.n_win; ++q) {
                const int len = w.hi[q] - w.lo[q] + 1, np = (len + piece_cols - 1) / piece_cols;
                for (int j = 0; j < np; ++j) {
                    const int own_lo = w.lo[q] + (int)((long)len * j / np), own_hi = w.lo[q] + (int)((long)len * (j + 1) / np) - 1;
                    AlignTask t = head;
                    const int start = std::max(0, own_lo - 1 - ov_w);
                    t.levels = head.levels + start; t.n = own_hi - start; t.col_off = start;
                    t.ckpt = reinterpret_cast<float*>((uintptr_t)ck2 * 4);
                    ck2 += (size_t)align_num_ckpts(t.n) * per_ckpt;
                    cols2 += t.n; out.wave_steps += align_num_steps(t.n); out.columns += t.n;
                    t2.push_back(t); ++made;
                }
                c->screen_stats[4] += len;
            }
            for (; made < need; ++made) { AlignTask t = head; t.n = 0; t.col_off = 0; t2.push_back(t); }
            g.lds = std::max(g.lds, p.tab_total[e.i]); g.known = g.known && in.m[e.i] == 870;
            pos_sorted.push_back(e.pos); grp_first.push_back(n_grp); n_grp += need / 4; ++slot;
        }
        g.n_grp = n_grp - g.first_grp;
        if (g.n_grp <= 0) continue;
        g.tables = tables_for(p, g.lds, 4);
        if (g.tables < 1) { c->err = "score table does not fit LDS"; return STRQ_ERR_UNSUPPORTED; }
        groups2.push_back(g);
    }
    grp_first.push_back(n_grp);
    c->look2_served += slot;
    if (slot > 0) {
        const size_t p_seg = 0, p_res = p_seg + (size_t)n_grp * 4 * sizeof(AlignResult), p_pick = p_res + (size_t)n_grp * sizeof(AlignResult),
                     p_first = p_pick + (size_t)n_grp * 4, p_pos = p_first + ((size_t)slot + 1) * 4, p_end = p_pos + (size_t)slot * 4;
        STRQ_HIP(c, c->ckpt2.reserve(ck2 * 4 + 256 + p_end + 256));
        char* rb = c->ckpt2.as<char>() + ((ck2 * 4 + 255) & ~(size_t)255);
        for (size_t x = 0; x < t2.size(); ++x) if (t2[x].n > 0) t2[x].ckpt = c->ckpt2.as<float>() + ((uintptr_t)t2[x].ckpt / 4);
        AlignResult* d_seg2 = reinterpret_cast<AlignResult*>(rb + p_seg); AlignResult* d_res2 = reinterpret_cast<AlignResult*>(rb + p_res);
        int32_t* d_pick2 = reinterpret_cast<int32_t*>(rb + p_pick);
        AlignTask* d_tasks2 = p.d_tasks + p.r2_0;
        STRQ_HIP(c, hipMemcpyAsync(d_tasks2, t2.data(), t2.size() * sizeof(AlignTask), hipMemcpyHostToDevice, st));
        STRQ_HIP(c, hipMemcpyAsync(rb + p_first, grp_first.data(), grp_first.size() * 4, hipMemcpyHostToDevice, st));
        STRQ_HIP(c, hipMemcpyAsync(rb + p_pos, pos_sorted.data(), (size_t)slot * 4, hipMemcpyHostToDevice, st));
        STRQ_HIP(c, hipMemsetAsync(d_seg2, 0, (size_t)n_grp * 4 * sizeof(AlignResult), st));
        for (const G2& g : groups2) {
            if (launch_align_segments(st, g.R, S, d_tasks2 + (size_t)g.first_grp * 4, d_seg2 + (size_t)g.first_grp * 4, g.n_grp, 4, c->queue.as<int>() + p.qi,
                                      c->ap, g.lds, g.tables, c->n_cu, 0, nullptr, nullptr, g.known)) { c->err = "align launch failed"; return STRQ_ERR_DEVICE; }
            ++p.qi; ++out.n_launches;
            if (launch_align_combine(st, d_tasks2 + (size_t)g.first_grp * 4, d_seg2 + (size_t)g.first_grp * 4, g.n_grp, 4, d_res2 + g.first_grp, d_pick2 + g.first_grp,
                                     (int)p.r2_0 + g.first_grp * 4)) { c->err = "combine launch failed"; return STRQ_ERR_DEVICE; }
        }
        if (launch_align_scatter(st, d_res2, d_pick2, reinterpret_cast<const int32_t*>(rb + p_first), reinterpret_cast<const int32_t*>(rb + p_pos), slot, p.d_res, p.d_pick)) { c->err = "scatter launch failed"; return STRQ_ERR_DEVICE; }
    }
    const bool forced = p.scr_forced || p.mode_coarse || c->screen_mode_last == 1;
    if (p.coarse_all > 0 && (p.coarse_cols + cols2 > 0.30 * p.coarse_all || 3 * n2 > nb) && nb >= 64 && !forced && c->coarse_pause == 0) pause_after_fail(c->coarse_pause, c->coarse_fail);
    STRQ_DBG("coarse screen, second look: %d alignments, %.2f %% of the columns (first look %.2f %%) -> pause %d", slot, 100.0 * cols2 / std::max(1.0, p.coarse_all), 100.0 * p.coarse_cols / std::max(1.0, p.coarse_all), c->coarse_pause);
    return STRQ_OK;
}

static int second_look(CorePlan& p, bool allow_bail, bool* bailed)
{
    if (!p.screen2_ran || !p.any_two_round || p.r2_cap <= 0) return STRQ_OK;
    strq_ctx* c = p.c; const AlignCoreOut& out = p.out;
    const int nb = p.nb;
    hipStream_t st = p.st;
    const std::vector<Launch>& launches = p.launches;
    std::vector<std::vector<int>> redo_keep(launches.size());
    std::vector<int> cnt(launches.size()), hredo((size_t)nb);
    std::vector<AlignResult> hres((size_t)nb);
    STRQ_HIP(c, hipMemcpyAsync(cnt.data(), p.d_redo_count, launches.size() * 4, hipMemcpyDeviceToHost, st));
    STRQ_HIP(c, hipMemcpyAsync(hredo.data(), p.d_redo, (size_t)nb * 4, hipMemcpyDeviceToHost, st));
    STRQ_HIP(c, hipMemcpyAsync(hres.data(), p.d_res, (size_t)nb * sizeof(AlignResult), hipMemcpyDeviceToHost, st));
    STRQ_HIP(c, hipStreamSynchronize(st));
    std::vector<Look2> l2;
    bool any_redo = false;
    for (size_t li = 0; li < launches.size(); ++li) {
        if (!p.two_round[li]) continue;
        const Launch& L = launches[li];
        for (int x = 0; x < cnt[li]; ++x) {
            const int a = hredo[(size_t)L.first + x], pos = L.first + a, i = out.order[pos];
            any_redo = true;
            if (p.g2_of[i] >= 0 && p.wins[i].n_win > 0 && (int)l2.size() < p.r2_cap && L.NS == 1) l2.push_back({pos, i, p.g2_of[i], hres[(size_t)pos].best});
            else redo_keep[li].push_back(a);
        }
    }
    size_t n_redo = l2.size();
    for (auto& v : redo_keep) n_redo += v.size();
    const bool forced = p.scr_forced || p.mode_coarse || c->screen_mode_last == 1;
    if (allow_bail && !forced && nb >= 64 && 3 * n_redo > (size_t)nb && !strq::opt("STRQ_SCREEN2_NO_BAIL")) {
        pause_after_fail(c->coarse_pause, c->coarse_fail);
        float ms = 0;
        STRQ_HIP(c, hipEventRecord(c->ev[3], st));
        STRQ_HIP(c, hipStreamSynchronize(st));
        STRQ_HIP(c, hipEventElapsedTime(&ms, c->ev[2], c->ev[3])); c->aborted_fwd_ms += ms;
        STRQ_HIP(c, hipEventElapsedTime(&ms, c->ev[5], c->ev[6])); c->aborted_screen_ms += ms;
        c->look2_served += (int64_t)n_redo;
        STRQ_DBG("coarse screen: %zu of %d alignments missed the first look's certificate -> the sub-batch starts over with the fine screen, pause %d", n_redo, nb, c->coarse_pause);
        *bailed = true;
        return STRQ_OK;
    }
    if (!l2.empty()) {
        const int rc = look2_run(p, l2, redo_keep);
        if (rc) return rc;
    }
    if (any_redo) {
        std::vector<int> redo_keep_n(launches.size(), 0);
        for (size_t li = 0; li < launches.size(); ++li) {
            if (!p.two_round[li]) continue;
            redo_keep_n[li] = (int)redo_keep[li].size();
            if (!redo_keep[li].empty()) STRQ_HIP(c, hipMemcpyAsync(p.d_redo + launches[li].first, redo_keep[li].data(), redo_keep[li].size() * 4, hipMemcpyHostToDevice, st));
        }
        STRQ_HIP(c, hipMemcpyAsync(p.d_redo_count, redo_keep_n.data(), launches.size() * 4, hipMemcpyHostToDevice, st));
    }
    return STRQ_OK;
}

static int second_round_and_trace(CorePlan& p)
{
    strq_ctx* c = p.c; AlignCoreOut& out = p.out;
    const int S = p.S;
    hipStream_t st = p.st;
    const std::vector<Launch>& launches = p.launches;
    for (size_t li = 0; li < launches.size(); ++li) {
        const Launch& L = launches[li];
        int* redo = p.d_redo + L.first; int* cnt = p.d_redo_count + li;
        if (!p.two_round[li]) continue;
        if (launch_align_segments(st, L.R, S, p.d_tasks + p.safe0 + L.first_task, p.d_seg_safe + L.first_task, L.count, L.segs, c->queue.as<int>() + p.qi,
                                  c->ap, L.lds_floats, L.tables, c->n_cu, L.packed, redo, cnt, L.known_last_row)) { c->err = "align launch failed"; return STRQ_ERR_DEVICE; }
        ++p.qi;
        if (launch_align_combine(st, p.d_tasks + p.safe0 + L.first_task, p.d_seg_safe + L.first_task, L.count, L.segs, p.d_res + L.first, p.d_pick + L.first,
                                 (int)p.safe0 + L.first_task, redo, cnt, nullptr, nullptr, nullptr)) { c->err = "combine launch failed"; return STRQ_ERR_DEVICE; }
    }
    STRQ_HIP(c, hipEventRecord(c->ev[3], st));
    for (size_t li = 0; li < launches.size();) {
        const Launch& L = launches[li];
        int count = L.count, lds_floats = L.lds_floats;
        size_t lj = li + 1;
        for (; lj < launches.size(); ++lj) {
            const Launch& M = launches[lj];
            if (M.R != L.R || M.NS != L.NS || M.packed != L.packed || L.NS != 1 || M.first != L.first + count) break;
            count += M.count; lds_floats = std::max(lds_floats, M.lds_floats);
        }
        const int wpb = std::min(trace_wpb, (160 * 1024) / (std::max(lds_floats, 1) * 4));
        if (launch_align(st, L.R, S, p.d_tasks, p.d_res + L.first, count, c->queue.as<int>() + p.qi, c->ap, lds_floats, wpb, c->n_cu,
                         c->scratch.as<uint64_t>(), 1, 0, L.packed, p.d_pick + L.first)) { c->err = "trace launch failed"; return STRQ_ERR_DEVICE; }
        ++p.qi; li = lj;
    }
    STRQ_HIP(c, hipEventRecord(c->ev[4], st));
    out.d_tasks = p.d_heads; out.d_results = p.d_res; out.d_rec = c->rec.as<int32_t>();
    return STRQ_OK;
}

static int align_core_once(strq_ctx* c, const AlignCoreIn& in, AlignCoreOut& out, bool allow_bail, bool* bailed)
{
    CorePlan p(c, in, out);
    int rc;
    if ((rc = upload_inputs(p))) return rc;
    if ((rc = build_tables(p))) return rc;
    read_switches(p);
    if ((rc = run_screens(p))) return rc;
    if ((rc = plan_launches(p))) return rc;
    if ((rc = cut_pieces(p))) return rc;
    if ((rc = write_tasks(p))) return rc;
    if ((rc = run_forward(p))) return rc;
    bool bail = false;
    if ((rc = second_look(p, allow_bail, &bail))) return rc;
    if (bail) { *bailed = true; return STRQ_OK; }
    return second_round_and_trace(p);
}

int align_core(strq_ctx* c, const AlignCoreIn& in, AlignCoreOut& out)
{
    double saved[8];
    std::memcpy(saved, c->screen_stats, sizeof(saved));
    bool bailed = false;
    const int rc = align_core_once(c, in, out, true, &bailed);
    if (rc || !bailed) return rc;
    std::memcpy(c->screen_stats, saved, sizeof(saved));
    return align_core_once(c, in, out, false, &bailed);
}

int align_core_times(strq_ctx* c, float* t_lut, float* t_fwd, float* t_tr)
{
    float ms;
    STRQ_HIP(c, hipEventElapsedTime(&ms, c->ev[0], c->ev[1])); *t_lut += ms;
    STRQ_HIP(c, hipEventElapsedTime(&ms, c->ev[2], c->ev[3])); *t_fwd += ms + c->aborted_fwd_ms;
    c->screen_stats[0] += c->aborted_screen_ms;
    c->aborted_fwd_ms = c->aborted_screen_ms = 0;
    STRQ_HIP(c, hipEventElapsedTime(&ms, c->ev[3], c->ev[4])); *t_tr += ms;
    if (c->screen_ran) { STRQ_HIP(c, hipEventElapsedTime(&ms, c->ev[5], c->ev[6])); c->screen_stats[0] += ms; }
    return STRQ_OK;
}

size_t align_workspace_bytes(int n, int m, int R, int NS)
{
    size_t b = (size_t)NS * (align_num_ckpts(n) + align_num_ckpts(n) / 4 + 300) * STRQ_CKPT_FIELDS(R) * 64 * 4;
    if (NS > 1) b += (size_t)(NS - 1) * ((size_t)n + 2) * 8;
    (void)m;
    return b;
}

int align_validate_flank(strq_ctx* c, const float* f, int64_t mm, int samples, int* k_out, int* R_out, int* NS_out)
{
    if (mm < 1 || samples < 1 || mm % samples != 0) { c->err = "flank length must be a positive multiple of `samples`"; return STRQ_ERR_UNSUPPORTED; }
    for (int64_t i = 0; i < mm; ++i)
        if (std::memcmp(&f[i], &f[i - i % samples], 4) != 0) { c->err = "flank is not made of runs of `samples` equal values"; return STRQ_ERR_UNSUPPORTED; }
    const int S = align_effective_samples(samples);
    int R = 0, NS = 0;
    if (mm > (1 << 20) || !align_plan((int)mm, S, &R, &NS)) { c->err = "flank shape not covered by the compiled kernels"; return STRQ_ERR_UNSUPPORTED; }
    if (S == 6 && mm / S > STRQ_LUT_MAX_K && NS == 1) { R = 12; NS = (int)((mm + 64 * 12 - 1) / (64 * 12)); }
    *k_out = (int)(mm / S); *R_out = R; *NS_out = NS;
    return STRQ_OK;
}

static int run_align_batch(strq_ctx* c, const BatchIn& in, const BatchOut& out)
{
    const int S = align_effective_samples(in.samples);
    const int64_t NA = in.n_align;
    std::fill(c->timing, c->timing + 8, 0.0f);
    for (double& v : c->screen_stats) v = 0;
    if (NA == 0) return STRQ_OK;
    std::vector<int> m(NA), k(NA), R(NA), n(NA), NS(NA);
    for (int64_t a = 0; a < NA; ++a) {
        const int64_t mm = in.flank_off[a + 1] - in.flank_off[a];
        const int rd = in.align_read[a];
        if (rd < 0 || rd >= in.n_reads) { c->err = "align_read out of range"; return STRQ_ERR_ARG; }
        const int64_t nn = in.read_off[rd + 1] - in.read_off[rd];
        if (nn < 0 || nn > (int64_t)1 << 30) { c->err = "bad read length"; return STRQ_ERR_ARG; }
        const int rc = align_validate_flank(c, in.flank + in.flank_off[a], mm, in.samples, &k[a], &R[a], &NS[a]);
        if (rc) return rc;
        m[a] = (int)mm; n[a] = (int)nn;
    }
    hipStream_t st = c->stream;
    c->second_round[0] = 0; c->second_round[1] = NA; c->look2_served = 0;
    STRQ_HIP(c, c->redo_total.reserve(64));
    STRQ_HIP(c, hipMemsetAsync(c->redo_total.p, 0, 64, st));
    const int64_t tot_levels = in.read_off[in.n_reads];
    STRQ_HIP(c, c->levels.reserve((size_t)tot_levels + 64));
    STRQ_HIP(c, c->level_val.reserve((size_t)in.n_reads * 256 * 4));
    STRQ_HIP(c, hipMemcpyAsync(c->levels.p, in.levels, (size_t)tot_levels, hipMemcpyHostToDevice, st));
    STRQ_HIP(c, hipMemcpyAsync(c->level_val.p, in.level_val, (size_t)in.n_reads * 256 * 4, hipMemcpyHostToDevice, st));
    int64_t a0 = 0;
    float t_lut = 0, t_fwd = 0, t_tr = 0, n_hard = 0, n_launch = 0;
    std::fill(c->counters, c->counters + 8, 0.0);
    while (a0 < NA) {
        int64_t a1 = a0; size_t ck_bytes = 0;
        while (a1 < NA) {
            const size_t need = align_workspace_bytes(n[a1], m[a1], R[a1], NS[a1]);
            if (a1 > a0 && ck_bytes + need > c->max_ws_bytes) break;
            ck_bytes += need; ++a1;
        }
        const int nb = (int)(a1 - a0);
        AlignCoreIn ci; AlignCoreOut co;
        ci.nb = nb; ci.samples = S; ci.d_levels = c->levels.as<uint8_t>(); ci.read_off = in.read_off;
        ci.d_level_val = c->level_val.as<float>();
        std::vector<const float*> fl(nb);
        for (int i = 0; i < nb; ++i) fl[i] = in.flank + in.flank_off[a0 + i];
        ci.read = in.align_read + a0; ci.n = &n[a0]; ci.m = &m[a0]; ci.k = &k[a0]; ci.R = &R[a0]; ci.NS = &NS[a0]; ci.flank = fl.data();
        int rc = align_core(c, ci, co);
        if (rc) return rc;
        std::vector<AlignResult> res(nb);
        std::vector<int32_t> h_rec(co.rec_total);
        STRQ_HIP(c, hipMemcpyAsync(res.data(), co.d_results, (size_t)nb * sizeof(AlignResult), hipMemcpyDeviceToHost, st));
        if (out.rec) STRQ_HIP(c, hipMemcpyAsync(h_rec.data(), co.d_rec, co.rec_total * 4, hipMemcpyDeviceToHost, st));
        STRQ_HIP(c, hipStreamSynchronize(st));
        for (int pos = 0; pos < nb; ++pos) {
            const int i = co.order[pos]; const int64_t a = a0 + i;
            if (out.score) out.score[a] = res[pos].best;
            if (out.j_end) out.j_end[a] = res[pos].j_end;
            if (out.j0) out.j0[a] = res[pos].j0;
            if (out.rec) std::memcpy(out.rec + in.flank_off[a], &h_rec[co.rec_off[i]], (size_t)m[a] * 4);
        }
        rc = align_core_times(c, &t_lut, &t_fwd, &t_tr);
        if (rc) return rc;
        n_hard += co.n_hard; n_launch += co.n_launches;
        c->counters[0] += co.wave_steps; c->counters[1] += co.columns; c->counters[2] += nb;
        c->counters[3] = co.segs; c->counters[4] = co.tables; c->counters[5] = co.packed; c->counters[6] = co.rows_per_lane;
        a0 = a1;
    }
    c->timing[0] = t_lut; c->timing[1] = t_fwd; c->timing[2] = t_tr; c->timing[3] = t_lut + t_fwd + t_tr; c->timing[4] = n_hard; c->timing[7] = n_launch;
    {
        unsigned int redo = 0;
        STRQ_HIP(c, hipMemcpy(&redo, c->redo_total.p, 4, hipMemcpyDeviceToHost));
        c->second_round[0] = (int64_t)redo - c->look2_served;
    }
    return STRQ_OK;
}

}

extern "C" {

int strq_abi_version(void) { return 12; }

int strq_set_option(strq_ctx* c, const char* key, const char* value)
{
    if (!key || std::strncmp(key, "STRQ_", 5) != 0) { if (c) c->err = "option keys start with STRQ_"; return STRQ_ERR_ARG; }
    if (c) { std::lock_guard<std::mutex> lk(c->options_mu); if (value) c->options[key] = value; else c->options.erase(key); return STRQ_OK; }
    std::lock_guard<std::mutex> lk(g_opt_mu);
    if (value) g_opts[key] = value; else g_opts.erase(key);
    return STRQ_OK;
}

int strq_get_option(const strq_ctx* c, const char* key, char* out, int32_t cap)
{
    if (!key || !out || cap < 1) return STRQ_ERR_ARG;
    CtxScope scope(c);
    const char* v = opt(key);
    out[0] = 0;
    if (!v) return STRQ_OK;
    std::strncpy(out, v, (size_t)cap - 1); out[cap - 1] = 0;
    return STRQ_OK;
}

int strq_ctx_create(int device_id, strq_ctx** out)
{
    if (!out) return STRQ_ERR_ARG;
    *out = nullptr;
    int ndev = 0;
    if (hipGetDeviceCount(&ndev) != hipSuccess || ndev <= 0 || device_id < 0 || device_id >= ndev) return STRQ_ERR_DEVICE;
    if (hipSetDevice(device_id) != hipSuccess) return STRQ_ERR_DEVICE;
    strq_ctx* c = new strq_ctx();
    c->device = device_id;
    hipDeviceProp_t prop;
    if (hipGetDeviceProperties(&prop, device_id) != hipSuccess) { delete c; return STRQ_ERR_DEVICE; }
    c->n_cu = prop.multiProcessorCount;
    if (hipStreamCreateWithFlags(&c->stream, hipStreamNonBlocking) != hipSuccess) { delete c; return STRQ_ERR_DEVICE; }
    for (auto& e : c->ev) if (hipEventCreate(&e) != hipSuccess) { delete c; return STRQ_ERR_DEVICE; }
    *out = c;
    return STRQ_OK;
}

void strq_ctx_destroy(strq_ctx* c)
{
    if (!c) return;
    (void)hipSetDevice(c->device);
    if (c->stream) (void)hipStreamSynchronize(c->stream);
    detect_state_free(c);
    for (DevBuf* b : {&c->levels, &c->level_val, &c->flank_cls, &c->tables, &c->tables3, &c->band_lo, &c->col0, &c->ckpt,
                      &c->rec, &c->tasks, &c->results, &c->queue, &c->scratch, &c->lutinfo, &c->hard, &c->misc,
                      &c->vit_x, &c->vit_tasks, &c->vit_bp, &c->vit_path, &c->bnd, &c->gen_codes, &c->gen_table, &c->gen_bnd, &c->gen_trace, &c->gen_hard, &c->redo_total, &c->screen, &c->ckpt2})
        b->release();
    for (HostModel* m : c->models) if (m) { m->blob.release(); delete m; }
    for (auto& e : c->ev) if (e) (void)hipEventDestroy(e);
    if (c->ev_fork) (void)hipEventDestroy(c->ev_fork);
    if (c->side_join) (void)hipEventDestroy(c->side_join);
    if (c->side_stream) (void)hipStreamDestroy(c->side_stream);
    if (c->stream) (void)hipStreamDestroy(c->stream);
    delete c;
}

const char* strq_last_error(const strq_ctx* c) { return c ? c->err.c_str() : "null context"; }

int strq_set_align_params(strq_ctx* c, const float p[6])
{
    if (!c || !p) return STRQ_ERR_ARG;
    c->ap = AlignParams{p[0], p[1], p[2], p[3], p[4], p[5]};
    return STRQ_OK;
}
int strq_get_align_params(const strq_ctx* c, float p[6])
{
    if (!c || !p) return STRQ_ERR_ARG;
    p[0] = c->ap.open_h; p[1] = c->ap.ext_h; p[2] = c->ap.open_v; p[3] = c->ap.ext_v;
    p[4] = c->ap.dist_offset; p[5] = c->ap.dist_min;
    return STRQ_OK;
}

int strq_device_synchronize(strq_ctx* c)
{
    if (!c) return STRQ_ERR_ARG;
    STRQ_HIP(c, hipSetDevice(c->device));
    STRQ_HIP(c, hipDeviceSynchronize());
    return STRQ_OK;
}

int strq_last_timing(const strq_ctx* c, float ms[8])
{
    if (!c || !ms) return STRQ_ERR_ARG;
    std::memcpy(ms, c->timing, sizeof(c->timing));
    return STRQ_OK;
}

int strq_last_counters(const strq_ctx* c, double out[8])
{
    if (!c || !out) return STRQ_ERR_ARG;
    std::memcpy(out, c->counters, sizeof(c->counters));
    return STRQ_OK;
}

int strq_debug_screen_plan(const float params[6], int32_t samples, int32_t max_n, int32_t out[6])
{
    if (!params || !out) return 0;
    const AlignParams p{params[0], params[1], params[2], params[3], params[4], params[5]};
    ScreenParams sp;
    if (!screen_plan(p, samples, max_n, &sp)) return 0;
    out[0] = sp.sc; out[1] = sp.hh; out[2] = sp.v; out[3] = sp.cadd; out[4] = sp.slack; out[5] = sp.merge_gap;
    return 1;
}

int strq_last_overlap(const strq_ctx* c, double out[4])
{
    if (!c || !out) return STRQ_ERR_ARG;
    for (int i = 0; i < 4; ++i) out[i] = c->overlap[i];
    return STRQ_OK;
}
int strq_last_screen(const strq_ctx* c, double out[8])
{
    if (!c || !out) return STRQ_ERR_ARG;
    for (int i = 0; i < 8; ++i) out[i] = c->screen_stats[i];
    return STRQ_OK;
}

int strq_last_screen_mode(const strq_ctx* c, int32_t out[8])
{
    if (!c || !out) return STRQ_ERR_ARG;
    for (int i = 0; i < 8; ++i) out[i] = 0;
    out[0] = c->screen_mode_last; out[1] = c->coarse_pause; out[2] = c->screen_pause; out[3] = (int32_t)c->coarse_margin;
    out[5] = (int32_t)std::min<int64_t>(c->look2_served, INT32_MAX);
    out[4] = c->screen_mode_last ? c->coarse_merge_last : 0;
    return STRQ_OK;
}

int strq_last_second_round(const strq_ctx* c, int64_t out[2])
{
    if (!c || !out) return STRQ_ERR_ARG;
    out[0] = c->second_round[0]; out[1] = c->second_round[1];
    return STRQ_OK;
}

int strq_last_viterbi_launches(const strq_ctx* c, int32_t out[4])
{
    if (!c || !out) return STRQ_ERR_ARG;
    std::memcpy(out, c->vit_launches, sizeof(c->vit_launches));
    return STRQ_OK;
}

int strq_last_geometry(const strq_ctx* c, int32_t out[8])
{
    if (!c || !out) return STRQ_ERR_ARG;
    std::memcpy(out, c->geometry, sizeof(c->geometry));
    return STRQ_OK;
}

int strq_align_batch(strq_ctx* c, int64_t n_align, int64_t n_reads, const uint8_t* levels,
                     const int64_t* read_off, const float* level_val, const int32_t* align_read,
                     const float* flank, const int64_t* flank_off, int32_t samples,
                     float* score, int64_t* j_end, int64_t* j0, int32_t* rec)
{
    strq::CtxScope scope_(c);
    if (!c) return STRQ_ERR_ARG;
    if (n_align < 0 || n_reads < 0 || (n_align > 0 && (!levels || !read_off || !level_val || !align_read || !flank || !flank_off)) || samples < 1) {
        c->err = "bad argument"; return STRQ_ERR_ARG;
    }
    STRQ_HIP(c, hipSetDevice(c->device));
    BatchIn in{n_align, n_reads, levels, read_off, level_val, align_read, flank, flank_off, samples};
    BatchOut out{score, j_end, j0, rec};
    return run_align_batch(c, in, out);
}

static int align_overlap_generic(strq_ctx* c, const float* a, int64_t n, const float* b, int64_t m, float* score,
                                 std::vector<int32_t>& rec, int64_t* je, int64_t* j0)
{
    if (n > ((int64_t)1 << 30) || m > ((int64_t)1 << 24) || (double)(n + 1) * (double)(m + 1) > 1.7e10) {
        c->err = "align_overlap: (n + 1) x (m + 1) exceeds the 16 GiB trace limit of the generic path"; return STRQ_ERR_UNSUPPORTED;
    }
    hipStream_t st = c->stream;
    auto encode = [](const float* x, int64_t len, std::vector<float>& vals, std::vector<uint32_t>& code) {
        std::vector<uint32_t> bits((size_t)len);
        std::memcpy(bits.data(), x, (size_t)len * 4);
        std::vector<uint32_t> uniq(bits);
        std::sort(uniq.begin(), uniq.end());
        uniq.erase(std::unique(uniq.begin(), uniq.end()), uniq.end());
        code.resize((size_t)len);
        for (int64_t i = 0; i < len; ++i) code[(size_t)i] = (uint32_t)(std::lower_bound(uniq.begin(), uniq.end(), bits[(size_t)i]) - uniq.begin());
        vals.resize(uniq.size());
        std::memcpy(vals.data(), uniq.data(), uniq.size() * 4);
    };
    std::vector<float> va, vb; std::vector<uint32_t> ca, cb;
    encode(a, n, va, ca); encode(b, m, vb, cb);
    const size_t na = va.size(), nbv = vb.size();
    if ((double)na * (double)nbv > 2.0e9) { c->err = "align_overlap: more than 2e9 distinct (a, b) value pairs"; return STRQ_ERR_UNSUPPORTED; }
    const size_t tab = std::max<size_t>(1, na * nbv);
    const int hard_cap = 1 << 20;
    STRQ_HIP(c, c->gen_codes.reserve(((size_t)n + (size_t)m + na + nbv) * 4 + 64));
    STRQ_HIP(c, c->gen_table.reserve(tab * 4 + 64));
    STRQ_HIP(c, c->gen_bnd.reserve(((size_t)n + 1) * 16 + ((size_t)m + 1) * 4 + 256));
    STRQ_HIP(c, c->gen_trace.reserve(((size_t)n + 1) * ((size_t)m + 1) + 64));
    STRQ_HIP(c, c->gen_hard.reserve((size_t)hard_cap * (sizeof(GenericHard) + 4) + 64));
    STRQ_HIP(c, c->results.reserve(sizeof(AlignResult) + 64));
    STRQ_HIP(c, c->queue.reserve(STRQ_QUEUE_BYTES));
    uint32_t* d_ca = c->gen_codes.as<uint32_t>(); uint32_t* d_cb = d_ca + n;
    float* d_va = reinterpret_cast<float*>(d_cb + m); float* d_vb = d_va + na;
    float* d_tab = c->gen_table.as<float>();
    float* d_bnd = c->gen_bnd.as<float>();
    GenericHard* d_hard = c->gen_hard.as<GenericHard>(); float* d_hvals = reinterpret_cast<float*>(d_hard + hard_cap);
    int* d_count = c->queue.as<int>();
    if (n) STRQ_HIP(c, hipMemcpyAsync(d_ca, ca.data(), (size_t)n * 4, hipMemcpyHostToDevice, st));
    STRQ_HIP(c, hipMemcpyAsync(d_cb, cb.data(), (size_t)m * 4, hipMemcpyHostToDevice, st));
    if (na) STRQ_HIP(c, hipMemcpyAsync(d_va, va.data(), na * 4, hipMemcpyHostToDevice, st));
    STRQ_HIP(c, hipMemcpyAsync(d_vb, vb.data(), nbv * 4, hipMemcpyHostToDevice, st));
    STRQ_HIP(c, hipMemsetAsync(d_count, 0, 4, st));
    int hard_count = 0;
    if (na) {
        if (launch_generic_table(st, d_va, (int)na, d_vb, (int)nbv, d_tab, d_hard, d_count, hard_cap, c->ap)) { c->err = "table launch failed"; return STRQ_ERR_DEVICE; }
        STRQ_HIP(c, hipMemcpyAsync(&hard_count, d_count, 4, hipMemcpyDeviceToHost, st));
        STRQ_HIP(c, hipStreamSynchronize(st));
        if (hard_count > hard_cap) {
            std::vector<float> full(tab);
            for (size_t y = 0; y < nbv; ++y) for (size_t x = 0; x < na; ++x) full[y * na + x] = host_cell_score(c->ap, va[x], vb[y]);
            STRQ_HIP(c, hipMemcpy(d_tab, full.data(), tab * 4, hipMemcpyHostToDevice));
        } else if (hard_count > 0) {
            std::vector<GenericHard> he((size_t)hard_count); std::vector<float> hv((size_t)hard_count);
            STRQ_HIP(c, hipMemcpy(he.data(), d_hard, (size_t)hard_count * sizeof(GenericHard), hipMemcpyDeviceToHost));
            for (int i = 0; i < hard_count; ++i) hv[(size_t)i] = host_cell_score(c->ap, va[(size_t)he[(size_t)i].ia], vb[(size_t)he[(size_t)i].ib]);
            STRQ_HIP(c, hipMemcpyAsync(d_hvals, hv.data(), (size_t)hard_count * 4, hipMemcpyHostToDevice, st));
            if (launch_generic_patch(st, d_tab, (int)na, d_hard, d_hvals, hard_count)) { c->err = "patch launch failed"; return STRQ_ERR_DEVICE; }
        }
    }
    c->timing[4] = (float)hard_count;
    std::vector<float> col0((size_t)m + 1);
    host_col0(c->ap, (int)m, col0.data());
    GenericAlignArgs ga;
    ga.code_a = d_ca; ga.code_b = d_cb; ga.table = d_tab;
    ga.bnd_S[0] = d_bnd; ga.bnd_V[0] = d_bnd + (n + 1); ga.bnd_S[1] = d_bnd + 2 * (n + 1); ga.bnd_V[1] = d_bnd + 3 * (n + 1);
    float* d_col0 = d_bnd + 4 * (n + 1);
    STRQ_HIP(c, hipMemcpyAsync(d_col0, col0.data(), ((size_t)m + 1) * 4, hipMemcpyHostToDevice, st));
    ga.col0 = d_col0; ga.trace = c->gen_trace.as<uint8_t>(); ga.result = c->results.as<AlignResult>();
    ga.p = c->ap; ga.n = (int32_t)n; ga.m = (int32_t)m; ga.na = (int32_t)na; ga.nb = (int32_t)nbv;
    if (launch_generic_align(st, ga)) { c->err = "generic align launch failed"; return STRQ_ERR_DEVICE; }
    AlignResult res;
    std::vector<uint8_t> trace(((size_t)n + 1) * ((size_t)m + 1));
    STRQ_HIP(c, hipMemcpyAsync(&res, ga.result, sizeof(res), hipMemcpyDeviceToHost, st));
    STRQ_HIP(c, hipMemcpyAsync(trace.data(), ga.trace, trace.size(), hipMemcpyDeviceToHost, st));
    STRQ_HIP(c, hipStreamSynchronize(st));
    rec.assign((size_t)m, 0);
    int64_t i = m, j = res.j_end; int state = 0;
    const size_t W = (size_t)n + 1;
    while (i > 0 && j > 0) {
        const uint8_t tr = trace[(size_t)i * W + (size_t)j];
        if (state == 0) {
            const unsigned dsel = tr & 3u;
            if (dsel == 0) { rec[(size_t)i - 1] = (int32_t)(j << 1); --i; --j; }
            else state = (int)dsel;
        } else if (state == 1) { --j; if (!(tr & 4u)) state = 0; }
        else { rec[(size_t)i - 1] = (int32_t)((j << 1) | 1); --i; if (!(tr & 8u)) state = 0; }
    }
    for (; i > 0; --i) rec[(size_t)i - 1] = (int32_t)((j << 1) | 1);
    *score = res.best; *je = res.j_end; *j0 = j;
    return STRQ_OK;
}

int strq_align_overlap(strq_ctx* c, const float* a, int64_t n, const float* b, int64_t m, float* score,
                       uint64_t* a_idx, uint64_t* b_idx, int32_t* rec_out, int64_t* j_end_out, int64_t* j0_out)
{
    strq::CtxScope scope_(c);
    if (!c) return STRQ_ERR_ARG;
    if ((!a && n > 0) || !b || n < 0 || m < 1 || !score) { c->err = "bad argument"; return STRQ_ERR_ARG; }
    STRQ_HIP(c, hipSetDevice(c->device));
    std::fill(c->timing, c->timing + 8, 0.0f);
    std::vector<int32_t> rec((size_t)m);
    int64_t je = 0, j0 = 0;
    std::vector<float> vals(a, a + n);
    std::sort(vals.begin(), vals.end(), [](float x, float y) { return __builtin_bit_cast(uint32_t, x) < __builtin_bit_cast(uint32_t, y); });
    vals.erase(std::unique(vals.begin(), vals.end(), [](float x, float y) { return std::memcmp(&x, &y, 4) == 0; }), vals.end());
    int run = 0;
    { int64_t start = 0;
      for (int64_t i = 1; i <= m; ++i)
          if (i == m || std::memcmp(&b[i], &b[start], 4) != 0) { int len = (int)std::min<int64_t>(i - start, 1 << 20); run = run ? std::__gcd(run, len) : len; start = i; } }
    bool fast = vals.size() <= 256 && run >= 1 && !strq::opt("STRQ_GENERIC_ALIGN");
    for (float v : vals) if (v != v) fast = false;
    if (fast) {
        std::sort(vals.begin(), vals.end());
        for (size_t x = 1; x < vals.size(); ++x) if (vals[x] == vals[x - 1]) fast = false;
        int kk, RR, NN;
        if (fast && align_validate_flank(c, b, m, run, &kk, &RR, &NN) != STRQ_OK) fast = false;
    }
    if (fast) {
        std::vector<uint8_t> lv((size_t)n);
        for (int64_t i = 0; i < n; ++i) lv[(size_t)i] = (uint8_t)(std::lower_bound(vals.begin(), vals.end(), a[i]) - vals.begin());
        std::vector<float> lval(256, INFINITY);
        std::copy(vals.begin(), vals.end(), lval.begin());
        const int64_t roff[2] = {0, n}, foff[2] = {0, m};
        const int32_t ar = 0;
        BatchIn in{1, 1, lv.data(), roff, lval.data(), &ar, b, foff, run};
        BatchOut out{score, &je, &j0, rec.data()};
        const int rc = run_align_batch(c, in, out);
        if (rc) return rc;
    } else {
        const int rc = align_overlap_generic(c, a, n, b, m, score, rec, &je, &j0);
        if (rc) return rc;
    }
    if (rec_out) std::memcpy(rec_out, rec.data(), (size_t)m * 4);
    if (j_end_out) *j_end_out = je;
    if (j0_out) *j0_out = j0;
    if (a_idx || b_idx) {
        if (a_idx) for (int64_t x = 0; x < j0; ++x) a_idx[x] = (uint64_t)x;
        int64_t ai = j0, col = j0;
        for (int64_t kk = 0; kk < m; ++kk) {
            const int64_t j = rec[(size_t)kk] >> 1; const bool vert = rec[(size_t)kk] & 1;
            const int64_t upto = vert ? j : j - 1;
            for (; ai < upto; ++ai, ++col) if (a_idx) a_idx[ai] = (uint64_t)col;
            if (b_idx) b_idx[kk] = (uint64_t)col;
            if (!vert) { if (a_idx) a_idx[ai] = (uint64_t)col; ++ai; }
            ++col;
        }
        for (; ai < n; ++ai, ++col) if (a_idx) a_idx[ai] = (uint64_t)col;
    }
    return STRQ_OK;
}

}
```

strique_amd/csrc/strq_ctx.h:

```cpp
#pragma once
#include <hip/hip_runtime.h>
#include <stdint.h>
#include <string>
#include <vector>
#include <map>
#include <cstdio>
#include <functional>
#include <mutex>
#include "align_kernels.h"
#include "viterbi_kernels.h"
#include "screen_kernels.h"
#include "strq_opt.h"

namespace strq {

struct DevBuf {
    void* p = nullptr;
    size_t cap = 0;
    hipError_t reserve(size_t bytes)
    {
        if (bytes <= cap) return hipSuccess;
        if (p) { (void)hipFree(p); p = nullptr; cap = 0; }
        size_t want = bytes + bytes / 8 + 256;
        hipError_t e = hipMalloc(&p, want);
        if (e == hipSuccess) cap = want;
        return e;
    }
    void release() { if (p) (void)hipFree(p); p = nullptr; cap = 0; }
    template <class T> T* as() const { return reinterpret_cast<T*>(p); }
};

#define STRQ_QUEUE_BYTES 65536
#define STRQ_QUEUE_FIRST 8
#define STRQ_QUEUE_SLOTS (STRQ_QUEUE_BYTES / 4)

struct AlignCoreIn {
    int nb = 0, samples = 6;
    const uint8_t* d_levels = nullptr;
    const int64_t* read_off = nullptr;
    const float* d_level_val = nullptr;
    const int32_t* read = nullptr;
    const int* n = nullptr; const int* m = nullptr; const int* k = nullptr; const int* R = nullptr;
    const int* NS = nullptr;
    const float* const* flank = nullptr;
    std::function<int()> after_tables;
};
struct AlignCoreOut {
    std::vector<int> order;
    std::vector<size_t> rec_off;
    size_t rec_total = 0;
    AlignTask* d_tasks = nullptr; AlignResult* d_results = nullptr; int32_t* d_rec = nullptr;
    int n_hard = 0;
    int n_launches = 0;
    double wave_steps = 0, columns = 0;
    int segs = 1, tables = 0, packed = 0, rows_per_lane = 0;
    int overlap_first = 0, overlap_worst = 0;
};

struct HostModel {
    VitModel h;
    const VitModel* dev = nullptr;
    DevBuf blob;
    DevBuf g2_blob;
    int32_t n_states = 0, silent_start = 0, start = 0, end = 0;
    std::vector<int32_t> in_ptr, in_src, emis_kind, count_inc, state_tag;
    std::vector<double> in_logp, emis_a, emis_b, emis_c;
};

}

struct strq_ctx {
    std::map<std::string, std::string> options;
    mutable std::mutex options_mu;
    int device = 0;
    int n_cu = 0;
    hipStream_t stream = nullptr;
    hipStream_t side_stream = nullptr;
    hipEvent_t ev_fork = nullptr, side_join = nullptr;
    hipEvent_t ev[8] = {};
    strq::AlignParams ap{-2.0f, -8.0f, -2.0f, -8.0f, 8.0f, -16.0f};
    std::string err;
    float timing[8] = {};
    double counters[8] = {};
    int32_t geometry[8] = {};
    int32_t vit_launches[4] = {};
    int64_t second_round[2] = {};
    strq::DevBuf redo_total;
    int64_t look2_served = 0;
    double screen_stats[8] = {};
    double overlap[4] = {};
    bool screen_ran = false;
    int screen_pause = 0;
    int coarse_pause = 0;
    int coarse_fail = 0, screen_fail = 0;
    float coarse_margin = 384.0f;
    float aborted_fwd_ms = 0, aborted_screen_ms = 0;
    int screen_mode_last = 0;
    int coarse_merge_last = 0;
    
    strq::DevBuf levels, level_val, flank_cls, tables, tables3, band_lo, col0, ckpt, rec, tasks, results,
        queue, scratch, lutinfo, hard, misc, vit_x, vit_tasks, vit_bp, vit_path, bnd,
        gen_codes, gen_table, gen_bnd, gen_trace, gen_hard,
        screen,
        ckpt2;
    std::vector<strq::HostModel*> models;
    void* detect = nullptr;
    size_t max_ws_bytes = (size_t)96 << 30;
    std::vector<float> score_fracs; double mean_n = 0;
};

namespace strq {
struct CtxScope { const strq_ctx* prev; explicit CtxScope(const strq_ctx* c); ~CtxScope(); };
int align_core(strq_ctx* c, const AlignCoreIn& in, AlignCoreOut& out);
int align_core_times(strq_ctx* c, float* t_lut, float* t_fwd, float* t_tr);
int align_validate_flank(strq_ctx* c, const float* f, int64_t m, int samples, int* k_out, int* R_out, int* NS_out);
size_t align_workspace_bytes(int n, int m, int R, int NS);
float host_cell_score(const AlignParams& p, float h, float v);
void detect_state_free(strq_ctx* c);
int detect_drain(strq_ctx* c);
int viterbi_launch_status(int vrc);
void host_stats_batch(const double* signals, const int64_t* offsets, int64_t n_reads, bool want_raw, double* out,
                      const double* const* reads = nullptr);
}

#define STRQ_ENTER(ctx)                                                                        \
    if (!(ctx)) return STRQ_ERR_ARG;                                                           \
    strq::CtxScope scope_(ctx);                                                                \
    STRQ_HIP(ctx, hipSetDevice((ctx)->device))

#define STRQ_HIP(ctx, call)                                                                    \
    do {                                                                                       \
        hipError_t e_ = (call);                                                                \
        if (e_ != hipSuccess) {                                                                \
            (ctx)->err = std::string(#call) + ": " + hipGetErrorString(e_);                    \
            return STRQ_ERR_DEVICE;                                                            \
        }                                                                                      \
    } while (0)
```

Before: 23360.

## Defer LUT table wait past screen upload and stage transfers through pinned host buffers

Measured after the change: 23490, median of 6. About the same (+0.5%).

```diff
diff --git a/strique_amd/csrc/screen_kernels.h b/strique_amd/csrc/screen_kernels.h
--- a/strique_amd/csrc/screen_kernels.h
+++ b/strique_amd/csrc/screen_kernels.h
@@ -62,6 +62,7 @@
 size_t screen2_lds_bytes(int tsize_a, int tsize_b);
 int launch_screen2(hipStream_t stream, const Screen2Task* tasks, int n_groups, int* queue, const ScreenParams& sp,
                    size_t lds_bytes, int groups_per_cu, int n_cu, int merge);
+int launch_screen2_table_sizes(hipStream_t stream, Screen2Task* tasks, int n_tasks, const int32_t* total, int stride);
 int launch_screen_windows(hipStream_t stream, const ScreenTask* tasks, int n_groups, const ScreenParams& sp,
                           const int32_t* bound_scaled, ScreenWindows* out, const int32_t* list = nullptr, const int32_t* theta_list = nullptr);
 
diff --git a/strique_amd/csrc/screen_kernels.hip b/strique_amd/csrc/screen_kernels.hip
--- a/strique_amd/csrc/screen_kernels.hip
+++ b/strique_amd/csrc/screen_kernels.hip
@@ -566,6 +566,22 @@
     return hipGetLastError() == hipSuccess ? 0 : 1;
 }
 
+__global__ void __launch_bounds__(256)
+screen2_table_sizes_kernel(Screen2Task* __restrict__ tasks, int n_tasks, const int32_t* __restrict__ total, int stride)
+{
+    const int x = blockIdx.x * blockDim.x + threadIdx.x;
+    if (x >= n_tasks) return;
+    tasks[x].tsize[0] = total[(size_t)tasks[x].tsize[0] * stride];
+    tasks[x].tsize[1] = total[(size_t)tasks[x].tsize[1] * stride];
+}
+
+int launch_screen2_table_sizes(hipStream_t stream, Screen2Task* tasks, int n_tasks, const int32_t* total, int stride)
+{
+    if (n_tasks <= 0) return 0;
+    hipLaunchKernelGGL(screen2_table_sizes_kernel, dim3((n_tasks + 255) / 256), dim3(256), 0, stream, tasks, n_tasks, total, stride);
+    return hipGetLastError() == hipSuccess ? 0 : 1;
+}
+
 int launch_screen(hipStream_t stream, const ScreenTask* tasks, int n_groups, int* queue, const ScreenParams& sp,
                   size_t lds_bytes, int tables_per_cu, int n_cu)
 {
diff --git a/strique_amd/csrc/strq_align_api.hip b/strique_amd/csrc/strq_align_api.hip
--- a/strique_amd/csrc/strq_align_api.hip
+++ b/strique_amd/csrc/strq_align_api.hip
@@ -124,6 +124,10 @@
     std::vector<float> h_cls;
     std::vector<LutJob> jobs;
     std::vector<LutInfo> info;
+    LutInfo* d_info = nullptr;
+    bool tables_waited = false;
+    int host_waits = 0;
+    double host_us[2] = {0, 0};
     std::vector<int> tab_total;
 
     std::vector<ScreenWindows> wins;
@@ -144,7 +148,8 @@
     std::vector<char> two_round;
     bool any_two_round = false;
     std::vector<size_t> ck_up;
-    std::vector<AlignTask> tasks;
+    AlignTask* tasks = nullptr;
+    size_t n_all_tasks = 0;
     AlignTask *d_tasks = nullptr, *d_heads = nullptr;
     AlignResult *d_seg = nullptr, *d_res = nullptr, *d_seg_safe = nullptr;
     int32_t* d_pick = nullptr;
@@ -245,16 +250,22 @@
     return STRQ_OK;
 }
 
-static int build_tables(CorePlan& p)
+static double now_us()
+{
+    timespec ts; clock_gettime(CLOCK_MONOTONIC, &ts);
+    return ts.tv_sec * 1e6 + ts.tv_nsec * 1e-3;
+}
+
+static int launch_tables(CorePlan& p)
 {
     strq_ctx* c = p.c; const AlignCoreIn& in = p.in;
-    const int nb = p.nb, nj = p.nj;
+    const int nj = p.nj;
     hipStream_t st = p.st;
     std::vector<LutJob>& jobs = p.jobs;
     std::vector<LutInfo>& info = p.info;
     jobs.resize(nj);
     LutJob* d_jobs = c->lutinfo.as<LutJob>();
-    LutInfo* d_info = reinterpret_cast<LutInfo*>(d_jobs + nj);
+    LutInfo* d_info = p.d_info = reinterpret_cast<LutInfo*>(d_jobs + nj);
     for (int j = 0; j < nj; ++j) {
         const int i = p.job_align[j];
         jobs[j].level_val = in.d_level_val + (size_t)in.read[i] * 256;
@@ -266,17 +277,35 @@
     }
     STRQ_HIP(c, hipMemcpyAsync(d_jobs, jobs.data(), (size_t)nj * sizeof(LutJob), hipMemcpyHostToDevice, st));
     HardEntry* d_hard = c->hard.as<HardEntry>();
-    float* d_hard_vals = reinterpret_cast<float*>(d_hard + hard_cap);
     int* d_hard_count = c->queue.as<int>();
     STRQ_HIP(c, hipEventRecord(c->ev[0], st));
     if (launch_lut_build(st, d_jobs, d_info, nj, p.max_k, d_hard, d_hard_count, hard_cap, c->ap)) { c->err = "lut launch failed"; return STRQ_ERR_DEVICE; }
     STRQ_HIP(c, hipEventRecord(c->ev[1], st));
     if (in.after_tables) { const int arc = in.after_tables(); if (arc) return arc; }
     info.resize(nj);
+    STRQ_HIP(c, c->pin_info.reserve((size_t)nj * sizeof(LutInfo) + 16));
+    STRQ_HIP(c, hipMemcpyAsync(c->pin_info.p, d_info, (size_t)nj * sizeof(LutInfo), hipMemcpyDeviceToHost, st));
+    STRQ_HIP(c, hipMemcpyAsync(c->pin_info.as<LutInfo>() + nj, d_hard_count, 4, hipMemcpyDeviceToHost, st));
+    return STRQ_OK;
+}
+
+static int wait_tables(CorePlan& p)
+{
+    if (p.tables_waited) return STRQ_OK;
+    p.tables_waited = true;
+    strq_ctx* c = p.c; const AlignCoreIn& in = p.in;
+    const int nb = p.nb, nj = p.nj;
+    hipStream_t st = p.st;
+    std::vector<LutJob>& jobs = p.jobs;
+    std::vector<LutInfo>& info = p.info;
+    LutJob* d_jobs = c->lutinfo.as<LutJob>();
+    HardEntry* d_hard = c->hard.as<HardEntry>();
+    float* d_hard_vals = reinterpret_cast<float*>(d_hard + hard_cap);
+    STRQ_HIP(c, hipStreamSynchronize(st)); ++p.host_waits;
+    p.host_us[0] = now_us();
+    std::memcpy(info.data(), c->pin_info.p, (size_t)nj * sizeof(LutInfo));
     int hard_count = 0;
-    STRQ_HIP(c, hipMemcpyAsync(info.data(), d_info, (size_t)nj * sizeof(LutInfo), hipMemcpyDeviceToHost, st));
-    STRQ_HIP(c, hipMemcpyAsync(&hard_count, d_hard_count, 4, hipMemcpyDeviceToHost, st));
-    STRQ_HIP(c, hipStreamSynchronize(st));
+    std::memcpy(&hard_count, c->pin_info.as<LutInfo>() + nj, 4);
     STRQ_DBG("lut done nb=%d hard=%d floats0=%d", nb, hard_count, info[0].total);
     if (strq::opt("STRQ_DEBUG")) { int hist[9] = {0}; for (int i = 0; i < nj; ++i) hist[std::min(8, info[i].need / 8)]++; STRQ_DBG("band need histogram (x8 levels): %d %d %d %d %d %d %d %d %d", hist[0], hist[1], hist[2], hist[3], hist[4], hist[5], hist[6], hist[7], hist[8]); }
     if (strq::opt("STRQ_DEBUG")) { long tot = 0; int mx = 0; for (int i = 0; i < nj; ++i) { tot += info[i].total; mx = std::max(mx, info[i].total); } STRQ_DBG("table floats: mean %.0f max %d (k=%d)", (double)tot / nj, mx, in.k[0]); }
@@ -298,7 +327,7 @@
         }
         STRQ_HIP(c, hipMemcpyAsync(d_hard_vals, hv.data(), (size_t)hard_count * 4, hipMemcpyHostToDevice, st));
         if (launch_lut_patch(st, d_jobs, d_hard, d_hard_vals, hard_count)) { c->err = "patch launch failed"; return STRQ_ERR_DEVICE; }
-        STRQ_HIP(c, hipStreamSynchronize(st));
+        STRQ_HIP(c, hipStreamSynchronize(st)); ++p.host_waits;
     }
     if (any_rebuild) for (int j = 0; j < nj; ++j) if (info[j].n_hard < 0) {
         const int kk = p.job_k[j], i = p.job_align[j];
@@ -314,9 +343,11 @@
         STRQ_HIP(c, hipMemcpy(jobs[j].band_lo, blo.data(), (size_t)kk * 4, hipMemcpyHostToDevice));
         info[j].total = kk * 256;
     }
+    if (any_rebuild) STRQ_HIP(c, hipMemcpy(p.d_info, info.data(), (size_t)nj * sizeof(LutInfo), hipMemcpyHostToDevice));
     p.tab_total.assign(nb, 0);
     for (int j = 0; j < nj; ++j) p.tab_total[p.job_align[j]] = std::max(p.tab_total[p.job_align[j]], info[j].total);
     p.out.n_hard = hard_count;
+    STRQ_HIP(c, hipEventRecord(c->ev[2], st));
     return STRQ_OK;
 }
 
@@ -374,7 +405,7 @@
         const int ov_worst = align_segment_overlap(p.c->ap, m_big), ov_s = overlap_for(p, m_big, ov_worst, 16);
         Piece pc[SSEG];
         const int used = cut(n, SSEG, ov_s, pc);
-        j.lds_bytes = std::max(j.lds_bytes, F == 2 ? screen2_lds_bytes(p.info[p.J0[a[0]]].total, p.info[p.J0[a[1]]].total) : screen_lds_bytes(p.info[p.J0[a[0]]].total));
+        if (F == 1) j.lds_bytes = std::max(j.lds_bytes, screen_lds_bytes(p.info[p.J0[a[0]]].total));
         for (int f = 0; f < F; ++f)
             j.bound[(size_t)g * F + f] = used <= 1 ? INT32_MIN / 2 : (ov_s >= ov_worst ? 0 : (int32_t)std::ceil((double)align_segment_min_score(p.c->ap, in.m[a[f]], ov_s) * sp.sc));
         for (int w = 0; w < SSEG; ++w) {
@@ -384,7 +415,7 @@
             t.n_chunks = pc[w].n > 0 ? (align_num_steps(pc[w].n) + 63) / 64 : 0;
             for (int f = 0; f < F; ++f) {
                 const LutJob& job = p.jobs[p.J0[a[f]]];
-                t.table[f] = job.table; t.band_lo[f] = job.band_lo; t.tsize[f] = p.info[p.J0[a[f]]].total; t.k[f] = in.k[a[f]];
+                t.table[f] = job.table; t.band_lo[f] = job.band_lo; t.tsize[f] = F == 2 ? p.J0[a[f]] : p.info[p.J0[a[f]]].total; t.k[f] = in.k[a[f]];
                 ScreenTask v; std::memset(&v, 0, sizeof(v));
                 v.n = pc[w].n; v.m = in.m[a[f]]; v.k = in.k[a[f]]; v.col_off = pc[w].col_off; v.n_chunks = t.n_chunks;
                 if (F == 2) v.lane_last = f * STRQ_SCREEN2_LANE_B + (in.k[a[f]] - 1) / STRQ_SCREEN2_CPL;
@@ -404,8 +435,6 @@
     strq_ctx* c = p.c; const AlignCoreIn& in = p.in;
     hipStream_t st = p.st;
     const int nv = (int)j.al.size();
-    if (j.lds_bytes > 160 * 1024 - 64) { c->err = r.lds_err; return STRQ_ERR_UNSUPPORTED; }
-    const int groups = std::max(1, std::min(r.groups_per_cu, (int)((160 * 1024 - 64) / j.lds_bytes)));
     auto aligned = [](size_t bytes) { return (bytes + 255) & ~(size_t)255; };
     const size_t t2_bytes = aligned(j.t2.size() * sizeof(Screen2Task)), task_bytes = aligned(j.views.size() * sizeof(ScreenTask));
     const size_t bound_bytes = aligned((size_t)nv * 4), win_bytes = aligned((size_t)nv * sizeof(ScreenWindows));
@@ -419,9 +448,21 @@
     for (size_t x = 0; x < j.views.size(); ++x) j.views[x].out = d_out + j.out_off[x];
     if (j.flanks == 2)
         for (int v = 0; v < nv; ++v) for (int w = 0; w < SSEG; ++w) j.t2[(size_t)(v / 2) * SSEG + w].out[v % 2] = j.views[(size_t)v * SSEG + w].out;
-    if (j.flanks == 2) STRQ_HIP(c, hipMemcpyAsync(d_t2, j.t2.data(), j.t2.size() * sizeof(Screen2Task), hipMemcpyHostToDevice, st));
-    STRQ_HIP(c, hipMemcpyAsync(d_st, j.views.data(), j.views.size() * sizeof(ScreenTask), hipMemcpyHostToDevice, st));
-    STRQ_HIP(c, hipMemcpyAsync(d_bound, j.bound.data(), (size_t)nv * 4, hipMemcpyHostToDevice, st));
+    const size_t up_bytes = t2_bytes + task_bytes + bound_bytes;
+    STRQ_HIP(c, c->pin_screen.reserve(up_bytes + win_bytes));
+    char* hb = c->pin_screen.as<char>();
+    if (j.flanks == 2) std::memcpy(hb, j.t2.data(), j.t2.size() * sizeof(Screen2Task));
+    std::memcpy(hb + t2_bytes, j.views.data(), j.views.size() * sizeof(ScreenTask));
+    std::memcpy(hb + t2_bytes + task_bytes, j.bound.data(), (size_t)nv * 4);
+    STRQ_HIP(c, hipMemcpyAsync(base, hb, up_bytes, hipMemcpyHostToDevice, st));
+    { const int rc = wait_tables(p); if (rc) return rc; }
+    if (j.flanks == 2) {
+        for (int g = 0; g < nv / 2; ++g)
+            j.lds_bytes = std::max(j.lds_bytes, screen2_lds_bytes(p.info[p.J0[j.al[(size_t)2 * g]]].total, p.info[p.J0[j.al[(size_t)2 * g + 1]]].total));
+        if (launch_screen2_table_sizes(st, d_t2, (int)j.t2.size(), &p.d_info->total, (int)(sizeof(LutInfo) / 4))) { c->err = "table sizes launch failed"; return STRQ_ERR_DEVICE; }
+    }
+    if (j.lds_bytes > 160 * 1024 - 64) { c->err = r.lds_err; return STRQ_ERR_UNSUPPORTED; }
+    const int groups = std::max(1, std::min(r.groups_per_cu, (int)((160 * 1024 - 64) / j.lds_bytes)));
     STRQ_HIP(c, hipEventRecord(c->ev[5], st));
     int* queue = c->queue.as<int>() + STRQ_QUEUE_FIRST - 1;
     if (j.flanks == 2) {
@@ -431,9 +472,11 @@
     }
     STRQ_HIP(c, hipEventRecord(c->ev[6], st));
     if (launch_screen_windows(st, d_st, nv, sp, d_bound, d_win)) { c->err = "screen windows launch failed"; return STRQ_ERR_DEVICE; }
-    std::vector<ScreenWindows> hw((size_t)nv);
-    STRQ_HIP(c, hipMemcpyAsync(hw.data(), d_win, hw.size() * sizeof(ScreenWindows), hipMemcpyDeviceToHost, st));
-    STRQ_HIP(c, hipStreamSynchronize(st));
+    p.host_us[0] = now_us() - p.host_us[0];
+    ScreenWindows* hw = reinterpret_cast<ScreenWindows*>(hb + up_bytes);
+    STRQ_HIP(c, hipMemcpyAsync(hw, d_win, (size_t)nv * sizeof(ScreenWindows), hipMemcpyDeviceToHost, st));
+    STRQ_HIP(c, hipStreamSynchronize(st)); ++p.host_waits;
+    p.host_us[1] = now_us();
     c->screen_ran = true; c->screen_mode_last = r.merge > 1 ? 2 : 1; c->coarse_merge_last = r.merge;
     if (const char* path = strq::opt("STRQ_SCREEN_DUMP")) {
         std::vector<int32_t> ho(j.out_words);
@@ -450,19 +493,19 @@
                     fwrite(th, 4, 4, fp);
                     fwrite(ho.data() + (t.out - d_out), 4, (size_t)t.n_chunks, fp);
                 }
-                fwrite(&hw[(size_t)v], sizeof(ScreenWindows), 1, fp);
+                fwrite(&hw[v], sizeof(ScreenWindows), 1, fp);
             }
             fclose(fp);
         }
     }
     if (const char* e = strq::opt("STRQ_SCREEN_TEST_RAISE")) {
         const float up = (float)atof(e);
-        for (auto& w : hw) w.lower_bound += up;
+        for (int v = 0; v < nv; ++v) hw[v].lower_bound += up;
     }
     int windowed = 0, heavy = 0, below_bound = 0; double cols = 0, all = 0;
     for (int v = 0; v < nv; ++v) {
         const int al = j.al[v];
-        const ScreenWindows& w = hw[(size_t)v];
+        const ScreenWindows& w = hw[v];
         c->screen_stats[1] += 1; c->screen_stats[7] += w.n_cand;
         double mine = in.n[al];
         if (w.n_win > 0) {
@@ -543,6 +586,7 @@
         if (in.NS[i] == 1 && p.NJ[i] == 1 && in.n[i] >= min_n && screen_flank_ok(in.m[i]) && in.k[i] * p.S == in.m[i]) sel.push_back(i);
     std::stable_sort(sel.begin(), sel.end(), [&](int x, int y) { return in.n[x] > in.n[y]; });
     if (sel.empty()) return STRQ_OK;
+    { const int rc = wait_tables(p); if (rc) return rc; }
     ScreenJob j;
     j.al = sel;
     screen_tasks(p, sp, j);
@@ -560,7 +604,6 @@
     const int nb = p.nb;
     p.wins.resize(nb);
     c->screen_ran = false;
-    STRQ_HIP(c, hipEventRecord(c->ev[2], p.st));
     int max_n = 0;
     for (int i = 0; i < nb; ++i) max_n = std::max(max_n, in.n[i]);
     c->screen_mode_last = 0;
@@ -659,15 +702,15 @@
         } else ++it;
     }
     out.order.clear(); out.order.reserve(nb);
+    std::vector<long> work((size_t)nb);
+    for (int x = 0; x < nb; ++x) {
+        long w = wins[x].n_win <= 0 ? (long)in.n[x] : 0;
+        for (int k = 0; k < wins[x].n_win; ++k) w += wins[x].hi[k] - wins[x].lo[k] + 1 + 4096;
+        work[(size_t)x] = w;
+    }
     for (auto& g : groups) {
         auto& v = g.second;
-        auto work = [&](int x) {
-            if (wins[x].n_win <= 0) return (long)in.n[x];
-            long w = 0;
-            for (int k = 0; k < wins[x].n_win; ++k) w += wins[x].hi[k] - wins[x].lo[k] + 1 + 4096;
-            return w;
-        };
-        std::stable_sort(v.begin(), v.end(), [&](int x, int y) { return work(x) > work(y); });
+        std::stable_sort(v.begin(), v.end(), [&](int x, int y) { return work[(size_t)x] > work[(size_t)y]; });
         const int NS = std::get<1>(g.first);
         const int pk = std::get<4>(g.first) == 0;
         int lds_floats = 0;
@@ -736,7 +779,10 @@
     p.r2_0 = n_all_tasks;
     STRQ_HIP(c, c->tasks.reserve((n_all_tasks + (size_t)p.r2_cap * 4) * sizeof(AlignTask)));
     STRQ_HIP(c, c->results.reserve((2 * n_tasks + nb) * sizeof(AlignResult) + (size_t)nb * 12 + p.launches.size() * 4 + 256));
-    p.tasks.resize(n_all_tasks);
+    p.n_all_tasks = n_all_tasks;
+    STRQ_HIP(c, c->pin_tasks.reserve(n_all_tasks * sizeof(AlignTask) + (size_t)nb * 4));
+    p.tasks = c->pin_tasks.as<AlignTask>();
+    std::memset(p.tasks, 0, n_all_tasks * sizeof(AlignTask));
     p.d_tasks = c->tasks.as<AlignTask>();
     p.d_heads = p.d_tasks + n_tasks + p.n_up;
     p.d_seg = c->results.as<AlignResult>();
@@ -749,43 +795,41 @@
     return STRQ_OK;
 }
 
+
+static AlignTask strip_task(const CorePlan& p, int i, int row0, int rows, size_t ck, int sidx)
+{
+    strq_ctx* c = p.c; const AlignCoreIn& in = p.in;
+    const int S = p.S;
+    AlignTask t; std::memset(&t, 0, sizeof(t));
+    t.levels = in.d_levels + in.read_off[in.read[i]];
+    t.rec = c->rec.as<int32_t>() + p.out.rec_off[i];
+    t.n = in.n[i]; t.n_full = in.n[i]; t.m_total = in.m[i];
+    const int j = p.NJ[i] > 1 ? p.J0[i] + sidx : p.J0[i];
+    const int k0 = row0 / S, k1 = (row0 + rows - 1) / S;
+    t.row0 = row0; t.m = rows; t.k = k1 - k0 + 1; t.tsize = p.info[j].total;
+    t.table = p.jobs[j].table; t.table3 = p.jobs[j].table3; t.band_lo = p.jobs[j].band_lo + (k0 - p.job_k0[j]);
+    t.col0 = c->col0.as<float>() + p.col0_off[i] + row0;
+    t.ckpt = c->ckpt.as<float>() + ck;
+    return t;
+}
+
 static int write_tasks(CorePlan& p)
 {
     strq_ctx* c = p.c; const AlignCoreIn& in = p.in; AlignCoreOut& out = p.out;
-    const int nb = p.nb, S = p.S;
+    const int nb = p.nb;
     hipStream_t st = p.st;
-    const size_t n_tasks = p.n_tasks, n_up = p.n_up, safe0 = p.safe0;
-    std::vector<AlignTask>& tasks = p.tasks;
+    const size_t n_tasks = p.n_tasks, n_up = p.n_up;
+    AlignTask* tasks = p.tasks;
     for (auto& L : p.launches) {
         for (int x = 0; x < L.count; ++x) {
             const int pos = L.first + x, i = out.order[pos];
             const int R = in.R[i], M = in.m[i];
-            AlignTask base; std::memset(&base, 0, sizeof(base));
-            base.levels = in.d_levels + in.read_off[in.read[i]];
-            base.rec = c->rec.as<int32_t>() + out.rec_off[i];
-            base.n = in.n[i]; base.n_full = in.n[i]; base.m_total = M;
-            auto strip = [&](int row0, int rows, size_t ck, int sidx) {
-                AlignTask t = base;
-                const int j = p.NJ[i] > 1 ? p.J0[i] + sidx : p.J0[i];
-                const int k0 = row0 / S, k1 = (row0 + rows - 1) / S;
-                t.row0 = row0; t.m = rows; t.k = k1 - k0 + 1; t.tsize = p.info[j].total;
-                t.table = p.jobs[j].table; t.table3 = p.jobs[j].table3; t.band_lo = p.jobs[j].band_lo + (k0 - p.job_k0[j]);
-                t.col0 = c->col0.as<float>() + p.col0_off[i] + row0;
-                t.ckpt = c->ckpt.as<float>() + ck;
-                return t;
-            };
-            tasks[n_tasks + n_up + pos] = strip(0, M, 0, 0);
             if (L.NS == 1) {
                 for (int k = 0; k < L.segs; ++k) {
                     const size_t ti = (size_t)L.first_task + (size_t)x * L.segs + k;
-                    AlignTask t = strip(0, M, p.pieces[ti].ck, 0);
+                    AlignTask t = strip_task(p, i, 0, M, p.pieces[ti].ck, 0);
                     t.levels += p.pieces[ti].col_off; t.n = p.pieces[ti].n; t.col_off = p.pieces[ti].col_off;
                     tasks[ti] = t;
-                    if (p.any_two_round) {
-                        AlignTask u = strip(0, M, p.safe[ti].ck, 0);
-                        u.levels += p.safe[ti].col_off; u.n = p.safe[ti].n; u.col_off = p.safe[ti].col_off;
-                        tasks[safe0 + ti] = u;
-                    }
                 }
             } else {
                 const int rows_s = 64 * R;
@@ -796,25 +840,52 @@
                     const bool last = sidx == L.NS - 1;
                     const int row0 = sidx * rows_s, rows = last ? M - row0 : rows_s;
                     const size_t slot = last ? (size_t)L.first_task + x : (size_t)L.first_up + (size_t)sidx * L.count + x;
-                    AlignTask t = strip(row0, rows, last ? p.pieces[(size_t)L.first_task + x].ck : p.ck_up[i] + (size_t)sidx * ck_strip, sidx);
+                    AlignTask t = strip_task(p, i, row0, rows, last ? p.pieces[(size_t)L.first_task + x].ck : p.ck_up[i] + (size_t)sidx * ck_strip, sidx);
                     if (sidx > 0) { t.bnd_in = bnd + (size_t)(sidx - 1) * bnd_stride; t.up = p.d_tasks + L.first_up + (size_t)(sidx - 1) * L.count + x; }
                     if (!last) t.bnd_out = bnd + (size_t)sidx * bnd_stride;
                     tasks[slot] = t;
-                    if (last && p.any_two_round) tasks[safe0 + slot] = t;
                 }
             }
         }
     }
-    STRQ_HIP(c, hipMemcpyAsync(p.d_tasks, tasks.data(), tasks.size() * sizeof(AlignTask), hipMemcpyHostToDevice, st));
+    STRQ_HIP(c, hipMemcpyAsync(p.d_tasks, tasks, (n_tasks + n_up) * sizeof(AlignTask), hipMemcpyHostToDevice, st));
     STRQ_HIP(c, hipMemsetAsync(p.d_seg, 0, (2 * n_tasks + nb) * sizeof(AlignResult), st));
-    if (p.any_two_round) {
-        STRQ_HIP(c, hipMemcpyAsync(p.d_min_score, p.min_score.data(), (size_t)nb * 4, hipMemcpyHostToDevice, st));
-        STRQ_HIP(c, hipMemsetAsync(p.d_redo_count, 0, p.launches.size() * 4, st));
-    }
+    if (p.any_two_round) STRQ_HIP(c, hipMemsetAsync(p.d_redo_count, 0, p.launches.size() * 4, st));
     size_t scratch_words = 0;
     for (auto& L : p.launches) scratch_words = std::max(scratch_words, align_trace_scratch_words_per_wave(L.R));
     STRQ_HIP(c, c->scratch.reserve(scratch_words * 8 * (size_t)c->n_cu * trace_wpb));
-    out.n_launches = 0; out.wave_steps = 0; out.columns = 0;
+    return STRQ_OK;
+}
+
+static int write_tasks_rest(CorePlan& p)
+{
+    strq_ctx* c = p.c; const AlignCoreIn& in = p.in; AlignCoreOut& out = p.out;
+    const int nb = p.nb;
+    hipStream_t st = p.st;
+    const size_t n_tasks = p.n_tasks, n_up = p.n_up, safe0 = p.safe0;
+    AlignTask* tasks = p.tasks;
+    for (auto& L : p.launches) {
+        for (int x = 0; x < L.count; ++x) {
+            const int pos = L.first + x, i = out.order[pos];
+            tasks[n_tasks + n_up + pos] = strip_task(p, i, 0, in.m[i], 0, 0);
+            if (!p.any_two_round) continue;
+            if (L.NS == 1) {
+                for (int k = 0; k < L.segs; ++k) {
+                    const size_t ti = (size_t)L.first_task + (size_t)x * L.segs + k;
+                    AlignTask u = strip_task(p, i, 0, in.m[i], p.safe[ti].ck, 0);
+                    u.levels += p.safe[ti].col_off; u.n = p.safe[ti].n; u.col_off = p.safe[ti].col_off;
+                    tasks[safe0 + ti] = u;
+                }
+            } else tasks[safe0 + (size_t)L.first_task + x] = tasks[(size_t)L.first_task + x];
+        }
+    }
+    STRQ_HIP(c, hipMemcpyAsync(p.d_tasks + n_tasks + n_up, tasks + n_tasks + n_up, (p.n_all_tasks - n_tasks - n_up) * sizeof(AlignTask), hipMemcpyHostToDevice, st));
+    if (p.any_two_round) {
+        float* h_min = reinterpret_cast<float*>(tasks + p.n_all_tasks);
+        std::memcpy(h_min, p.min_score.data(), (size_t)nb * 4);
+        STRQ_HIP(c, hipMemcpyAsync(p.d_min_score, h_min, (size_t)nb * 4, hipMemcpyHostToDevice, st));
+    }
+    out.wave_steps = 0; out.columns = 0;
     for (size_t t = 0; t < n_tasks + n_up; ++t) if (tasks[t].n > 0) { out.wave_steps += align_num_steps(tasks[t].n); out.columns += tasks[t].n; }
     if (!p.launches.empty()) {
         const Launch& L = p.launches.back(); out.segs = L.segs; out.tables = L.tables; out.packed = L.packed; out.rows_per_lane = L.R;
@@ -834,6 +905,7 @@
     hipStream_t st = p.st;
     const std::vector<Launch>& launches = p.launches;
     for (auto& L : launches) p.max_ns = std::max(p.max_ns, L.NS);
+    out.n_launches = 0;
     if ((size_t)STRQ_QUEUE_FIRST + launches.size() * ((size_t)p.max_ns + 2) + 16 > (size_t)STRQ_QUEUE_SLOTS) {
         c->err = "too many distinct (flank shape, table size) groups in one batch"; return STRQ_ERR_UNSUPPORTED;
     }
@@ -870,6 +942,8 @@
             ++p.qi; ++out.n_launches;
         }
     }
+    if (c->screen_ran) p.host_us[1] = now_us() - p.host_us[1];
+    { const int rc = write_tasks_rest(p); if (rc) return rc; }
     if (side) {
         STRQ_HIP(c, hipEventRecord(c->side_join, c->side_stream));
         STRQ_HIP(c, hipStreamWaitEvent(st, c->side_join, 0));
@@ -918,9 +992,9 @@
     STRQ_HIP(c, hipMemcpyAsync(mb + o_pos, h_pos.data(), (size_t)n2 * 4, hipMemcpyHostToDevice, st));
     if (launch_screen_windows(st, p.d_st2, n2, sp2, p.d_bound2, reinterpret_cast<ScreenWindows*>(mb + o_win),
                               reinterpret_cast<const int32_t*>(mb + o_list), reinterpret_cast<const int32_t*>(mb + o_theta))) { c->err = "screen windows launch failed"; return STRQ_ERR_DEVICE; }
-    std::vector<ScreenWindows> w2((size_t)n2);
-    STRQ_HIP(c, hipMemcpyAsync(w2.data(), mb + o_win, (size_t)n2 * sizeof(ScreenWindows), hipMemcpyDeviceToHost, st));
-    STRQ_HIP(c, hipStreamSynchronize(st));
+    const ScreenWindows* w2 = reinterpret_cast<const ScreenWindows*>(c->pin_look2.as<char>() + (size_t)nb * (sizeof(AlignResult) + 4) + p.launches.size() * 4);
+    STRQ_HIP(c, hipMemcpyAsync(const_cast<ScreenWindows*>(w2), mb + o_win, (size_t)n2 * sizeof(ScreenWindows), hipMemcpyDeviceToHost, st));
+    STRQ_HIP(c, hipStreamSynchronize(st)); ++p.host_waits;
     std::map<int, std::vector<int>> by_R;
     for (int k2 = 0; k2 < n2; ++k2) {
         if (w2[(size_t)k2].n_win > 0) by_R[in.R[l2[(size_t)k2].i]].push_back(k2);
@@ -1009,12 +1083,13 @@
     hipStream_t st = p.st;
     const std::vector<Launch>& launches = p.launches;
     std::vector<std::vector<int>> redo_keep(launches.size());
-    std::vector<int> cnt(launches.size()), hredo((size_t)nb);
-    std::vector<AlignResult> hres((size_t)nb);
-    STRQ_HIP(c, hipMemcpyAsync(cnt.data(), p.d_redo_count, launches.size() * 4, hipMemcpyDeviceToHost, st));
-    STRQ_HIP(c, hipMemcpyAsync(hredo.data(), p.d_redo, (size_t)nb * 4, hipMemcpyDeviceToHost, st));
-    STRQ_HIP(c, hipMemcpyAsync(hres.data(), p.d_res, (size_t)nb * sizeof(AlignResult), hipMemcpyDeviceToHost, st));
-    STRQ_HIP(c, hipStreamSynchronize(st));
+    STRQ_HIP(c, c->pin_look2.reserve((size_t)nb * (sizeof(AlignResult) + 4) + launches.size() * 4 + (size_t)p.r2_cap * sizeof(ScreenWindows)));
+    const AlignResult* hres = c->pin_look2.as<AlignResult>();
+    const int* hredo = reinterpret_cast<const int*>(hres + nb);
+    const int* cnt = hredo + nb;
+    STRQ_HIP(c, hipMemcpyAsync(c->pin_look2.p, p.d_res, (size_t)nb * sizeof(AlignResult), hipMemcpyDeviceToHost, st));
+    STRQ_HIP(c, hipMemcpyAsync(const_cast<int*>(hredo), p.d_redo, ((size_t)nb + launches.size()) * 4, hipMemcpyDeviceToHost, st));
+    STRQ_HIP(c, hipStreamSynchronize(st)); ++p.host_waits;
     std::vector<Look2> l2;
     bool any_redo = false;
     for (size_t li = 0; li < launches.size(); ++li) {
@@ -1034,7 +1109,7 @@
         pause_after_fail(c->coarse_pause, c->coarse_fail);
         float ms = 0;
         STRQ_HIP(c, hipEventRecord(c->ev[3], st));
-        STRQ_HIP(c, hipStreamSynchronize(st));
+        STRQ_HIP(c, hipStreamSynchronize(st)); ++p.host_waits;
         STRQ_HIP(c, hipEventElapsedTime(&ms, c->ev[2], c->ev[3])); c->aborted_fwd_ms += ms;
         STRQ_HIP(c, hipEventElapsedTime(&ms, c->ev[5], c->ev[6])); c->aborted_screen_ms += ms;
         c->look2_served += (int64_t)n_redo;
@@ -1099,15 +1174,18 @@
     CorePlan p(c, in, out);
     int rc;
     if ((rc = upload_inputs(p))) return rc;
-    if ((rc = build_tables(p))) return rc;
+    if ((rc = launch_tables(p))) return rc;
     read_switches(p);
     if ((rc = run_screens(p))) return rc;
+    if ((rc = wait_tables(p))) return rc;
     if ((rc = plan_launches(p))) return rc;
     if ((rc = cut_pieces(p))) return rc;
     if ((rc = write_tasks(p))) return rc;
     if ((rc = run_forward(p))) return rc;
     bool bail = false;
     if ((rc = second_look(p, allow_bail, &bail))) return rc;
+    if (c->screen_ran) STRQ_DBG("host waits inside align_core_once: %d; host time from the tables to the screen's launch %.0f us, from the windows to the first look's launches %.0f us", p.host_waits, p.host_us[0], p.host_us[1]);
+    else STRQ_DBG("host waits inside align_core_once: %d", p.host_waits);
     if (bail) { *bailed = true; return STRQ_OK; }
     return second_round_and_trace(p);
 }
@@ -1284,6 +1362,7 @@
                       &c->rec, &c->tasks, &c->results, &c->queue, &c->scratch, &c->lutinfo, &c->hard, &c->misc,
                       &c->vit_x, &c->vit_tasks, &c->vit_bp, &c->vit_path, &c->bnd, &c->gen_codes, &c->gen_table, &c->gen_bnd, &c->gen_trace, &c->gen_hard, &c->redo_total, &c->screen, &c->ckpt2})
         b->release();
+    for (HostBuf* b : {&c->pin_info, &c->pin_screen, &c->pin_tasks, &c->pin_look2}) b->release();
     for (HostModel* m : c->models) if (m) { m->blob.release(); delete m; }
     for (auto& e : c->ev) if (e) (void)hipEventDestroy(e);
     if (c->ev_fork) (void)hipEventDestroy(c->ev_fork);
diff --git a/strique_amd/csrc/strq_ctx.h b/strique_amd/csrc/strq_ctx.h
--- a/strique_amd/csrc/strq_ctx.h
+++ b/strique_amd/csrc/strq_ctx.h
@@ -27,6 +27,22 @@
         return e;
     }
     void release() { if (p) (void)hipFree(p); p = nullptr; cap = 0; }
+    template <class T> T* as() const { return reinterpret_cast<T*>(p); }
+};
+
+struct HostBuf {
+    void* p = nullptr;
+    size_t cap = 0;
+    hipError_t reserve(size_t bytes)
+    {
+        if (bytes <= cap) return hipSuccess;
+        if (p) { (void)hipHostFree(p); p = nullptr; cap = 0; }
+        size_t want = bytes + bytes / 8 + 256;
+        hipError_t e = hipHostMalloc(&p, want, hipHostMallocDefault);
+        if (e == hipSuccess) cap = want;
+        return e;
+    }
+    void release() { if (p) (void)hipHostFree(p); p = nullptr; cap = 0; }
     template <class T> T* as() const { return reinterpret_cast<T*>(p); }
 };
 
@@ -103,6 +119,10 @@
         gen_codes, gen_table, gen_bnd, gen_trace, gen_hard,
         screen,
         ckpt2;
+    strq::HostBuf pin_info,
+        pin_screen,
+        pin_tasks,
+        pin_look2;
     std::vector<strq::HostModel*> models;
     void* detect = nullptr;
     size_t max_ws_bytes = (size_t)96 << 30;
```
